# orottier/web-audio-api-rs

Hardware: NVIDIA H100
Metric: offline render-quanta/sec (48kHz stereo, 128-frame) (higher is better)
Workload: dtype f64 filter state / f32 PCM

## Files before the change

web-audio-api-rs_b200/csrc/wae_device.h:

```cpp
#pragma once
#include <cstdint>
#include <vector_types.h>

#include "wae_spatial.h"

namespace wae {

struct BufRef {
    float* p;
    uint32_t stride;
    uint32_t absolute;
    uint8_t* meta;
    uint32_t meta_stride;
    uint32_t meta_pad;
};
constexpr uint8_t WAE_META_SILENT = 0x80;

struct ChunkInfo {
    int64_t f0;
    int32_t nf;
    int32_t sub;
};

struct OscInst {
// ... 330 lines not shown
    float sample_rate;
    int32_t type;
    int32_t ch;
    int32_t pad;
    int32_t* dyn_len;
    BufRef coefs;
};

struct ParamEvDev {
    int32_t type;
    float value;
    double time;
    double aux;
    double cancel_time;
    int32_t has_cancel;
    int32_t values_off, values_len;
    int32_t pad;
};
struct ParamState {
    float intrinsic;
    int32_t head;
    int32_t has_last;
    int32_t override_valid;
    int32_t inited;
    int32_t pad;
    ParamEvDev last;
    ParamEvDev override_ev;
};
struct ParamInst {
    const ParamEvDev* events;
    const float* curves;
    ParamState* state;
    BufRef in;
    BufRef out;
    float def, mn, mx, intrinsic0;
    float sample_rate;
    int32_t n_events;
    int32_t a_rate;
    int32_t has_last0;
    ParamEvDev last0;
};

enum ChainSrc : int32_t { CHAIN_SRC_BUFFER = 0, CHAIN_SRC_ABSN = 1, CHAIN_SRC_OSC = 2, CHAIN_SRC_CONST = 3 };
struct ChainBiquad {
    double b0, b1, b2, a1, a2;
    double* state;
    int32_t coef;
    int32_t pad;
};
constexpr int CHAIN_MAX_BIQUADS = 2;
struct ChainInst {
    int32_t src_kind;
    int32_t ch;
    int32_t n_biquad;
    int32_t has_shaper;
    float g[4];
    int32_t out_dup;
    int32_t shaper_n;
    int32_t shaper_keeps_silence;
    int32_t pad2;
    const float* curve;
    BufRef in;
    AbsnInst absn;
    OscInst osc;
    ConstInst cst;
    BufRef out;
    int64_t limit;
    int64_t end;
    ChainBiquad bq[CHAIN_MAX_BIQUADS];
};

constexpr int CHAIN_MAX_SLABS = 64;
constexpr int CHAIN_MAX_PRE_SLABS = 256;
struct ChainSched {
    int32_t n_slabs;
    int32_t tiles_per_slab;
    int32_t max_ch;
    int32_t slab_stride;
    uint32_t epoch;
    int32_t pre_log2;
    unsigned* ticket;
    double* handoff;
    unsigned* flags;
};
struct ChainAux {
    unsigned* ticket = nullptr;
    double* handoff = nullptr;
    unsigned* flags = nullptr;
    int32_t slab_stride = 0;
    uint32_t epoch = 0;
};

struct VoiceGroup {
    int32_t first;
    int32_t n_voices;
    BufRef out;
    int32_t out_dup;
    int32_t pad;
    int64_t limit;
};

struct ConvInput {
    BufRef in;
    float* prev;
    float2* xring;
    int32_t in_channel;
    int32_t xring_blocks;
    int64_t end;
};
struct ConvPath {
    BufRef out;
    const float2* h;
    float2* y;
    int32_t input;
    int32_t S;
    int32_t out_channel;
    int32_t accumulate;
    int64_t limit;
    int64_t end;
};
struct ConvCmpInst {
    BufRef in;
    ConvInput x;
    ConvPath path;
    int64_t* cursor;
    float* carry;
    float* win;
    int32_t* qmap;
    int64_t* wdesc;
    int32_t in_ch;
    int32_t pad;
};

struct BindItem {
    float* dst;
    const float* src;
    int64_t stride;
    int64_t src_stride;
    int64_t len;
    int32_t channels;
    int32_t pad;
};

struct RespBindItem {
    const float* src;
    float2* h;
    int64_t src_stride;
    int64_t len;
    float sample_rate;
    int32_t channels;
    int32_t S;
    int32_t normalize;
    float scale;
    int32_t m[4];
    int32_t pad;
};

struct CurvePatch {
    int32_t* dst;
    int32_t keeps, other;
};
struct CurveBindItem {
    const float* src;
    float* dst;
    const CurvePatch* patches;
    int32_t n;
    int32_t n_patches;
};

struct WaveBindItem {
    const float* re;
    const float* im;
    float* dst;
// ... 152 lines not shown
```

web-audio-api-rs_b200/csrc/wae_engine.cu:

```cuda
#include "wae_graph.h"
#include "wae_hostmath.h"
#include "wae_hrtf_host.h"
#include "wae_resample_host.h"
#include "wae_kernels.h"
#include "wae_param_core.h"
#include "wae_param_host.h"

#include <cuda.h>
#include <cuda_runtime.h>
#include <emmintrin.h>

#include <algorithm>
#include <array>
#include <atomic>
#include <chrono>
#include <condition_variable>
#include <cstdlib>
#include <deque>
#include <fstream>
#include <mutex>
#include <sched.h>
#include <sstream>
#include <thread>
#include <cmath>
// ... 897 lines not shown
    std::vector<int> out_ch;
    std::vector<BufRef> out_buf;
    std::vector<Lay> out_lay;
    bool wrote_dest = false;
    Lay lay_out(int port) const { return port < (int)out_lay.size() ? out_lay[port] : Lay::fixed(out_ch[port]); }
};

struct NodeTable {
    std::vector<PNode> v;
    std::vector<char> has;
    void reset(uint32_t max_id) {
        if (v.size() < (size_t)max_id + 1) v.resize((size_t)max_id + 1);
        has.assign(v.size(), 0);
    }
    PNode& put(uint32_t id, Node* n) {
        if (id >= v.size()) {
            v.resize((size_t)id + 1);
            has.resize((size_t)id + 1, 0);
        }
        PNode& p = v[id];
        p.n = n;
        p.level = 0;
        p.in_edges.resize((size_t)n->n_inputs);
        for (auto& port : p.in_edges) port.clear();
        p.in_ch.clear();
        p.in_buf.clear();
        p.in_lay.clear();
        p.out_ch.clear();
        p.out_buf.clear();
        p.out_lay.clear();
        p.wrote_dest = false;
        has[id] = 1;
        return p;
    }
    PNode* find(uint32_t id) { return id < v.size() && has[id] ? &v[id] : nullptr; }
    bool count(uint32_t id) const { return id < v.size() && has[id]; }
    PNode& at(uint32_t id) {
        if (!(id < v.size() && has[id])) throw std::out_of_range("planner: unknown node id");
        return v[id];
    }
};

struct Planner {
    wae_batch* b;
    wae_engine* eng;
    Planner(wae_batch* b, const wae_batch::Group& grp, PrepState& ps, std::vector<wae_batch::Group::SrcCopy>* sizing_copies);
    std::map<std::pair<int, int>, StageBuild> builds;
    std::string error;
    int error_code = 0;
    uint64_t algorithmic_bytes = 0;
    struct IrSpectra {
        float2* h;
        int S;
        int channels;
    };
    std::unordered_map<uint64_t, IrSpectra> own_ir_cache;
    std::unordered_map<uint64_t, IrSpectra>* ir_cache = &own_ir_cache;
    std::map<int, std::pair<const float2*, const float2*>> os_filters;

    bool has_feedback = false;
    std::map<std::pair<uint32_t, uint32_t>, int>* delay_ch_hint = nullptr;
    std::map<std::pair<uint32_t, uint32_t>, int> delay_ch_seen;
    struct DelayRing {
        float* ring;
        uint32_t ring_len;
        int ch;
        int64_t* mono_at;
        int32_t mono_len;
    };
    std::map<std::pair<uint32_t, uint32_t>, DelayRing> delay_rings;
    std::map<std::pair<uint32_t, uint32_t>, int> conv_paths_seen;
    bool dry = false;
    int group_graphs = 1;
    int vs_mode = -1;
    int voice_sum_mode() {
        if (eng->voice_sum >= 0) return eng->voice_sum;
        if (vs_mode < 0) {
            const char* e = getenv("WAE_VOICE_SUM");
            vs_mode = e ? std::max(0, std::min(2, atoi(e))) : 0;
        }
        return vs_mode;
    }
    uint64_t arena_floats_per_frame = 0;
    float* d_src = nullptr;
    std::vector<wae_batch::Group::SrcCopy>* src_copies = nullptr;
    size_t src_cursor = 0;
    struct PendingChain {
        ChainInst inst;
        hm::BiquadCoefs coefs[CHAIN_MAX_BIQUADS] = {};
        int ch = 1;
        int phase = 0;
        int cls = 0;
        Lay lay;
        std::vector<Entry> entries;
        Entry gain_fold[4] = {};
        void add_entry(Entry e, size_t off, size_t field) {
            e.refer(0, T_A, -1, off, field);
            entries.push_back(e);
        }
    };

    uint32_t key_graph = 0, key_node = 0, key_seq = 0;
    uint64_t dry_gi = 0, dry_seq = 0;
    uintptr_t dry_addr() { return (uintptr_t)256 + ((dry_gi + 1) << 44) + (dry_seq++ << 24); }
    uint64_t key_salt = 0;
    template <typename T>
    T* alloc(size_t count, bool zero = false, bool rezero_on_run = false) {
        if (dry) return reinterpret_cast<T*>(dry_addr());
        if (seg_start == 0 && seg_end >= lq) return b->dalloc<T>(count, zero, rezero_on_run);
        const wae_batch::StateKey key{key_graph, key_node, key_seq++, key_salt};
        const size_t bytes = count * sizeof(T);
        std::lock_guard<std::recursive_mutex> lk(b->mu);
        auto it = b->state_map.find(key);
        if (it != b->state_map.end() && it->second.second == bytes) return (T*)it->second.first;
        T* p = b->dalloc<T>(count, zero, rezero_on_run);
        if (p) b->state_map[key] = {(void*)p, bytes};
        return p;
    }
    std::map<int, std::vector<float*>> arena_pool;
    std::map<int, size_t> arena_used;
    std::map<std::pair<uint32_t, uint32_t>, size_t> src_offsets;
    std::unordered_map<const PcmBuffer*, size_t> buf_offsets;
    struct ParamRecord {
        size_t n_source_events = 0;
        ParamTimeline tl;
        int64_t init_frame = 0;
    };
    std::unordered_map<uint64_t, ParamRecord> param_records;
    const ParamTimeline* param_timeline(uint32_t gi, uint32_t pid, const Param& prm, float sample_rate) {
        const uint64_t rec_key = (uint64_t)gi << 32 | pid;
        auto it = param_records.find(rec_key);
        if (it == param_records.end()) {
            ParamRecord r;
            r.tl = build_param_timeline(prm);
            r.n_source_events = prm.events.size();
            r.init_frame = seg_start;
            return &param_records.emplace(rec_key, std::move(r)).first->second.tl;
        }
        ParamRecord& r = it->second;
        if (r.n_source_events == prm.events.size() || !r.tl.error.empty()) return &r.tl;
        ParamInst host{};
        host.events = r.tl.events.data();
        host.curves = r.tl.curves.data();
        host.n_events = (int32_t)r.tl.events.size();
        host.a_rate = prm.a_rate ? 1 : 0;
        host.sample_rate = sample_rate;
        ParamState st{};
        st.intrinsic = r.tl.intrinsic;
        st.has_last = r.tl.has_last ? 1 : 0;
        st.last = r.tl.last;
        st.inited = 1;
        float buf[128];
        for (int64_t f = r.init_frame; f < seg_start; f += 128) param_compute_buffer(host, st, (double)f / (double)sample_rate, buf);
        ParamTimeline next;
        next.curves = r.tl.curves;
        for (int i = st.head; i < host.n_events; i++) next.events.push_back(i == st.head && st.override_valid ? st.override_ev : r.tl.events[i]);
        next.intrinsic = st.intrinsic;
        next.has_last = st.has_last != 0;
        next.last = st.last;
        fold_param_events(next, prm.events.data() + r.n_source_events, prm.events.size() - r.n_source_events);
        r.tl = std::move(next);
        r.n_source_events = prm.events.size();
        r.init_frame = seg_start;
        return &r.tl;
    }
    int64_t seg_start = 0, seg_end = 0;
    int64_t lq = 0, glq = 0;
    BufRef dest_ref() const { return BufRef{b->d_out + b->out_off[gi], (uint32_t)g->length, 1}; }
    void add_out(StageBuild& s, size_t off, int t = T_A) const {
        Entry e = entry(E_OUT);
        e.p.out.off = (uint64_t)b->out_off[gi];
        s.add_entry(e, off + offsetof(BufRef, p), offsetof(OutPatch, dst), t);
    }
    int64_t dest_reader = -1;
    void begin_segment(int64_t f0, int64_t f1) {
        seg_start = f0;
        seg_end = f1;
        builds.clear();
        arena_used.clear();
        arena_floats_per_frame = 0;
    }
    template <typename T>
    T* upload(const std::vector<T>& v) {
        if (dry) return reinterpret_cast<T*>(uintptr_t(256));
        return b->dupload(v);
    }

    bool bail(int code, const std::string& msg) {
        if (!error_code) {
            error_code = code;
            error = msg;
        }
        return false;
    }
    bool no_arena() { return bail(WAE_OUT_OF_MEMORY, "out of device memory (arena)"); }

    int cur_cls = 0;
    StageBuild& stage(int level, int kind, int variant = 0) {
        const int cls = cur_cls;
        const int order = kind >= S_READOUT_FFT ? S_ANALYSER * 64 - 3 + (kind - S_READOUT_FFT) : kind * 64 + variant;
        StageBuild& s = builds[{cls * 1000000 + level, order}];
        s.cls = cls;
        s.level = level;
        s.kind = kind;
        s.variant = variant;
        return s;
    }

    BufRef arena_buf(int ch, bool with_meta = false) {
        arena_floats_per_frame += (uint64_t)ch;
        const uint32_t mstride = (uint32_t)((b->chunk / 128 + 16) / 16 * 16);
        BufRef r{dry ? reinterpret_cast<float*>(dry_addr()) : nullptr, (uint32_t)b->chunk, 0, nullptr, 0, 0};
        if (!dry) {
            std::vector<float*>& pool = arena_pool[ch];
            size_t& used = arena_used[ch];
            if (used < pool.size()) {
                r.p = pool[used++];
            } else {
                const size_t floats = (size_t)ch * (size_t)b->chunk;
                float* p = b->dalloc<float>(floats + ((size_t)ch * mstride + 3) / 4);
                b->arena_bytes += floats * 4;
                if (p) {
                    pool.push_back(p);
                    used++;
                }
                r.p = p;
            }
        }
        if (with_meta && r.p) {
            r.meta = reinterpret_cast<uint8_t*>(r.p + (size_t)ch * (size_t)b->chunk);
            r.meta_stride = mstride;
        }
        return r;
    }
    void meta_stage(int L, int mode, const BufRef& in, int in_ch, const BufRef& out, int out_ch, int count = 0, int aux = 0) {
        MetaInst m{};
        m.in = in;
        m.out = out;
        m.mode = mode;
        m.in_ch = in_ch;
        m.out_ch = out_ch;
        m.count = count;
        m.aux = aux;
        stage(L, S_META).meta.push_back(m);
    }

    wae_graph* g = nullptr;
    uint32_t gi = 0;
    Orderer ord{};
    NodeTable node_table;
    SchedClock clock{48000.f};
    bool want_scan_coefs = false;
    std::map<uint32_t, PendingChain> pending;
    struct NodeCtx {
        uint32_t id;
        Node& n;
        PNode& p;
        int level = 0, L = 1;
        Lay in0;
        bool dyn_params = false, fuse_n = false;
        bool extend = false, dest_direct = false;
        uint32_t fuse_src = 0;
    };
// ... 970 lines not shown
        ch = max_in;
    }
    p.in_ch[port] = ch;
    p.in_lay[port] = Lay::fixed(ch);
    bool is_dest = n.kind == K_DEST;
    if (nc.extend || nc.dest_direct) {
        if (nc.extend) p.in_lay[port] = pending.at(nc.fuse_src).lay;
        return true;
    }
    if (vsum_nb >= 0) return sum_voices(nc, port, ch, vsum_nb);
    if (is_dest && edges.size() == 1 && pn.at(edges[0].node).wrote_dest) {
        p.in_buf[port] = pn.at(edges[0].node).out_buf[edges[0].port];
        return true;
    }
    bool any_dyn = false;
    Lay pl = Lay::fixed(ch);
    if (!edges.empty()) {
        int lo = 1, hi = 1, on_nlo = 0, min_nlo = 255;
        bool all_may_silent = true;
        for (auto& r : edges) {
            const Lay el = pn.at(r.node).lay_out(r.port);
            any_dyn = any_dyn || el.dyn();
            lo = std::max<int>(lo, el.lo);
            hi = std::max<int>(hi, el.hi);
            if (!el.may_silent) on_nlo = std::max<int>(on_nlo, el.nlo);
            min_nlo = std::min<int>(min_nlo, el.nlo);
            all_may_silent = all_may_silent && el.may_silent;
        }
        const int nlo = std::max(on_nlo, min_nlo);
        pl.lo = (uint8_t)computed_channels(n.cfg, lo);
        pl.hi = (uint8_t)computed_channels(n.cfg, hi);
        pl.nlo = (uint8_t)computed_channels(n.cfg, nlo);
        pl.nhi = pl.hi;
        pl.may_silent = all_may_silent;
        if (n.kind == K_DELAY_R) pl = pn.at(edges[0].node).lay_out(edges[0].port);
    }
    bool needs_fold = false;
    if (ch > 2 && n.cfg.mode != WAE_COUNT_MODE_EXPLICIT)
        for (auto& r : edges) needs_fold = needs_fold || pn.at(r.node).out_ch[r.port] != ch;
    if (!is_dest && edges.size() == 1 && pn.at(edges[0].node).out_ch[edges[0].port] == ch) {
        const Lay el = pn.at(edges[0].node).lay_out(edges[0].port);
        const bool identity = !el.dyn() || n.kind == K_DELAY_R || n.cfg.mode == WAE_COUNT_MODE_MAX ||
                              (n.cfg.mode == WAE_COUNT_MODE_CLAMPED_MAX && el.hi <= n.cfg.count);
        const bool canonical_needed = el.dyn() && n.kind == K_CONV;
        if (identity && !canonical_needed) {
            p.in_buf[port] = pn.at(edges[0].node).out_buf[edges[0].port];
            p.in_lay[port] = el;
            return true;
        }
    }
    const bool dyn = any_dyn || needs_fold;
    if (!mix(2 * nc.level, edges, ch, n.cfg, is_dest, dyn, dyn && pl.dyn(), p.in_buf[port])) return false;
    if (dyn) p.in_lay[port] = pl;
    return true;
}

bool Planner::sum_voices(NodeCtx& nc, int port, int ch, int nb) {
    auto& edges = nc.p.in_edges[port];
    StageBuild& vs = stage(2 * nc.level, S_VSUM, nb);
    VoiceGroup vg{};
    vg.first = (int32_t)vs.chain.size();
    vg.n_voices = (int32_t)edges.size();
    vg.out_dup = ch;
    vg.limit = -1;
    if (nc.n.kind == K_DEST) {
        vg.out = dest_ref();
        vg.limit = (int64_t)g->length;
    } else {
        vg.out = arena_buf(ch);
        if (!vg.out.p) return no_arena();
    }
    for (auto& r : edges) {
        PendingChain pc = std::move(pending.at(r.node));
        pending.erase(r.node);
        if (pc.inst.n_biquad == 1 && vs.n_scan_coef != vs.chain.size()) return bail(WAE_UNSUPPORTED, "internal: voice-sum coefficient table out of step");
        for (int k = 0; k < pc.inst.n_biquad; k++)
            pc.inst.bq[k].coef = vs.add_scan_coef(want_scan_coefs, [&] { return make_scan_coef(pc.coefs[k]); });
        pc.inst.limit = -1;
        pc.inst.out_dup = 0;
        chain_entries(vs, pc, (int32_t)vs.chain.size());
        vs.chain.push_back(pc.inst);
    }
    vs.vgroups.push_back(vg);
    if (nc.n.kind == K_DEST) add_out(vs, offsetof(VoiceGroup, out), T_C);
    nc.p.in_buf[port] = vg.out;
    return true;
}

bool Planner::lower_dest(NodeCtx& nc) {
    PNode& p = nc.p;
    p.out_ch = {(int)g->channels};
    if (nc.dest_direct) {
        PendingChain pc = std::move(pending.at(nc.fuse_src));
        pending.erase(nc.fuse_src);
        const BufRef fin = dest_ref();
        pc.inst.out = fin;
        pc.inst.limit = (int64_t)g->length;
        pc.inst.out_dup = (pc.ch == 1 && g->channels == 2) ? 2 : 0;
        add_out(emit_chain(pc, nc.L), offsetof(ChainInst, out));
        node_table.at(nc.fuse_src).out_buf = {fin};
        p.in_buf[0] = fin;
    }
    p.out_buf = {p.in_buf[0]};
    if (const std::vector<Edge>* outs = ord.edges.find(nc.id))
        for (auto& e : *outs)
            if (e.other_index >= 0 && dest_reader < 0) dest_reader = gi;
    algorithmic_bytes += (uint64_t)g->channels * g->length * 4;
    return true;
}

bool Planner::lower_osc(NodeCtx& nc) {
    Node& n = nc.n; PNode& p = nc.p;
    const double sr = (double)g->sample_rate;
    PRef pf = param_ref(n.params[0]), pd = param_ref(n.params[1]);
    float freq = pf.v, detune = pd.v;
    if (!nc.fuse_n && !need_out(nc, 1)) return false;
    OscInst o{};
    double start_ratio = 0.;
    if (!nc.fuse_n) o.out = p.out_buf[0];
    o.type = n.type;
    double computed_freq = (double)freq * std::exp2((double)detune / 1200.);
    o.incr = computed_freq / sr;
    o.inv_incr = o.incr != 0. ? 1. / o.incr : 0.;
    o.outside_nyquist = std::fabs(computed_freq) >= sr / 2.;
    o.n_first = std::numeric_limits<int64_t>::max();
    o.n_stop = std::numeric_limits<int64_t>::max();
    o.phase0 = 0.;
    if (n.start_time < 1e300) {
        const OscStart st = osc_start(clock, n.start_time, o.incr, o.outside_nyquist);
        o.n_first = st.n_first;
        o.phase0 = st.phase0;
        start_ratio = st.start_ratio;
        o.n_stop = osc_stop_frame(clock, n.stop_time);
    }
    SchedPatch sched{};
    if (n.device_schedule) sched = sched_entry(n, nc.dyn_params ? SCHED_OSC_AR : SCHED_OSC);
    SchedPatch meta_sched = sched;
    meta_sched.kind = SCHED_META_OSC;
    const SchedPatch* track_sched = n.device_schedule ? &meta_sched : nullptr;
    const bool pitch_bound = pf.bound >= 0 || pd.bound >= 0;
    Entry pitch = patch(PATCH_OSC, 2);
    if (pitch_bound && !nc.dyn_params) {
        const double f_lo = pf.bound >= 0 ? pf.lo : freq, f_hi = pf.bound >= 0 ? pf.hi : freq;
        const double d_lo = pd.bound >= 0 ? pd.lo : detune, d_hi = pd.bound >= 0 ? pd.hi : detune;
        if (!hm::osc_pitch_inside(f_lo, f_hi, d_lo, d_hi, sr)) {
            const uint32_t caller = b->order.empty() ? gi : b->order[gi];
            return bail(WAE_UNSUPPORTED, "graph " + std::to_string(caller) + ", OscillatorNode " + std::to_string(n.id) +
                                             ": the pitch bound from device memory allows computed frequencies outside (0, sampleRate / 2) "
                                             "with frequency [" + std::to_string(f_lo) + ", " + std::to_string(f_hi) + "] Hz and detune [" +
                                             std::to_string(d_lo) + ", " + std::to_string(d_hi) +
                                             "] cents (bind a wider pitch as a value curve: wae_param_set_device_value_curve)");
        }
        operand(pitch, 0, pf, freq);
        operand(pitch, 1, pd, detune);
        pitch.p.param.sample_rate = g->sample_rate;
        double* start = upload(std::vector<double>{n.start_time});
        if (!start) return bail(WAE_OUT_OF_MEMORY, "out of device memory (oscillator start time)");
        pitch.p.param.dst2 = start;
        if (n.device_schedule) sched.start_out = start;
    }
    if (n.type == WAE_OSC_CUSTOM && n.device_wave) {
        o.table = device_wave(n);
        o.table_len = (int)n.device_wave_len;
        if (!o.table) return false;
    } else if (n.type == WAE_OSC_CUSTOM) {
        float* d = upload(n.table);
// ... 1526 lines not shown
    }
    if (uniform) return WAE_OK;
    std::vector<std::vector<int64_t>> cuts(n_graphs);
    for (uint32_t i = 0; i < n_graphs; i++) cuts[i] = graph_cuts(graphs[i]);
    order.resize(n_graphs);
    for (uint32_t i = 0; i < n_graphs; i++) order[i] = i;
    std::stable_sort(order.begin(), order.end(), [&](uint32_t x, uint32_t y) {
        if (graphs[x]->sample_rate != graphs[y]->sample_rate) return graphs[x]->sample_rate < graphs[y]->sample_rate;
        if (cuts[x] != cuts[y]) return cuts[x] < cuts[y];
        return padded_length(graphs[x]) > padded_length(graphs[y]);
    });
    return WAE_OK;
}

static wae_status prep_begin(wae_engine* eng, wae_graph* const* graphs, uint32_t n_graphs, wae_plan_info* plan, wae_batch** out_b, PrepState& ps,
                             bool want_d_out, const std::vector<uint32_t>* order = nullptr) {
    if (!eng || !graphs || n_graphs == 0) return fail(WAE_INVALID_ARGUMENT, "null / empty batch");
    if (!plan) CUDA_TRY(cudaSetDevice(eng->device));
    for (uint32_t i = 0; i < n_graphs; i++) {
        if (!graphs[i]) return fail(WAE_INVALID_ARGUMENT, "null graph in the batch");
        if (!order && (graphs[i]->channels != graphs[0]->channels || graphs[i]->length != graphs[0]->length ||
                       graphs[i]->sample_rate != graphs[0]->sample_rate))
            return fail(WAE_INVALID_ARGUMENT, "all graphs of a batch must share number_of_channels, length and sample_rate");
    }
    ps.t0 = std::chrono::steady_clock::now();
    auto* b = new wae_batch;
    b->engine = eng;
    b->s_h2d = eng->s_h2d;
    b->s_d2h = eng->s_d2h;
    b->n_graphs = n_graphs;
    b->channels = graphs[0]->channels;
    b->out_off.assign(n_graphs + 1, 0);
    for (uint32_t i = 0; i < n_graphs; i++) {
        b->length = std::max(b->length, graphs[i]->length);
        b->out_off[i + 1] = b->out_off[i] + (size_t)graphs[i]->channels * graphs[i]->length;
        b->shape.push_back({graphs[i]->channels, graphs[i]->length});
    }
    b->lq = (int64_t)((b->length + 127) / 128 * 128);
    for (uint32_t i = 0; i < n_graphs; i++) b->needed_quanta += (uint64_t)(padded_length(graphs[i]) / 128);
    if (order) {
        b->mixed = true;
        b->order = *order;
        b->pos.assign(n_graphs, 0);
        for (uint32_t i = 0; i < n_graphs; i++) b->pos[b->order[i]] = i;
    }
    bool has_conv = false, has_hrtf = false;
    std::vector<char> graph_has_conv(n_graphs, 0);
    std::vector<std::vector<int64_t>> cuts(n_graphs);
    for (uint32_t i = 0; i < n_graphs; i++) {
        for (auto& kv : graphs[i]->nodes) {
            if (kv.second.kind == K_CONV && kv.second.buffer) graph_has_conv[i] = 1;
            if (kv.second.kind == K_PANNER && kv.second.panning_model == WAE_PANNING_HRTF) has_hrtf = true;
        }
        cuts[i] = graph_cuts(graphs[i]);
        for (auto& ep : graphs[i]->epochs)
            for (auto& kv : ep.nodes)
                if (kv.second.kind == K_CONV && kv.second.buffer) graph_has_conv[i] = 1;
        has_conv = has_conv || graph_has_conv[i];
    }
    size_t out_floats = b->out_off[n_graphs];
    if (!plan && want_d_out) {
        b->d_out = b->dalloc<float>(out_floats, true);
        if (!b->d_out) {
            wae_batch_destroy(b);
            return fail(WAE_OUT_OF_MEMORY, "out of device memory (output PCM)");
        }
    }
    b->groups = form_groups(eng, graphs, n_graphs, cuts);
    int n_groups = (int)b->groups.size();
    for (auto& grp : b->groups) {
        bool conv = false;
        for (uint32_t i = grp.g0; i < grp.g1; i++) conv = conv || graph_has_conv[i];
        if (!conv) continue;
        for (int64_t f : grp.seg_bounds)
            if (f != grp.lq && f % WAE_CONV_BLOCK != 0) {
                wae_batch_destroy(b);
                return fail(WAE_UNSUPPORTED, "a suspend point that is not a multiple of the convolver partition (8192 frames) in a graph with a ConvolverNode is not lowered to the GPU");
            }
    }
    b->chunk = 2048;
    uint64_t fpf = 0;
    bool has_feedback = false;
    std::vector<std::vector<int>> plan_stage_lists;
    struct SizeOut {
        uint64_t fpf = 0;
        bool has_feedback = false;
        std::map<std::pair<uint32_t, uint32_t>, int> delay_ch_seen;
        std::vector<std::vector<int>> stage_lists;
        uint64_t digest = 1469598103934665603ull, entries_digest = 1469598103934665603ull;
        size_t n_entries = 0;
        int code = WAE_OK;
        std::string error;
    };
    WorkerPool* pool = (!plan && n_groups > 1 && n_graphs >= 64) ? eng->workers() : nullptr;
    bool converged = false;
    for (int iter = 0; iter < 8; iter++) {
        bool hints_changed = false;
        fpf = 0;
        plan_stage_lists.clear();
        std::vector<SizeOut> so(n_groups);
        struct RangeOut {
            uint64_t fpf = 0;
            size_t src_floats = 0;
            bool has_feedback = false;
            std::map<std::pair<uint32_t, uint32_t>, int> delay_ch_seen;
            std::vector<wae_batch::Group::SrcCopy> copies;
            std::vector<size_t> graph_base;
            Builds builds;
            int code = WAE_OK;
            std::string error;
        };
        auto size_range = [&](int k, uint32_t i0, uint32_t i1, RangeOut& ro, size_t cursor0) {
            Planner sizing(b, b->groups[k], ps, &ro.copies);
            sizing.src_cursor = cursor0;
            sizing.begin_segment(0, b->groups[k].lq);
            for (uint32_t i = i0; i < i1; i++) {
                EpochView view(graphs[i], 0);
                ro.graph_base.push_back(sizing.src_cursor);
                if (!sizing.plan_graph(graphs[i], i)) {
                    ro.code = sizing.error_code;
                    ro.error = sizing.error;
                    return;
                }
            }
            if (plan) ro.builds = std::move(sizing.builds);
            ro.fpf = sizing.arena_floats_per_frame;
            ro.src_floats = sizing.src_cursor - cursor0;
            ro.has_feedback = sizing.has_feedback;
            ro.delay_ch_seen = std::move(sizing.delay_ch_seen);
        };
        auto size_group_split = [&](int k, WorkerPool* wp, int parts, RangeOut& out, const std::vector<size_t>* known_base = nullptr) {
            const uint32_t g0 = b->groups[k].g0, n = b->groups[k].g1 - g0;
            std::vector<RangeOut> ro((size_t)parts);
            auto run = [&](int t) {
                const uint32_t i0 = (uint32_t)((uint64_t)n * t / parts), i1 = (uint32_t)((uint64_t)n * (t + 1) / parts);
                size_range(k, g0 + i0, g0 + i1, ro[t], known_base ? (*known_base)[i0] : 0);
            };
            if (wp) wp->parallel_for(parts, run);
            else
                for (int t = 0; t < parts; t++) run(t);
            for (auto& r : ro) {
                if (r.code != WAE_OK) {
                    out.code = r.code;
                    out.error = r.error;
                    return false;
                }
                const size_t rebase = known_base ? 0 : out.src_floats;
                for (auto& c : r.copies) out.copies.push_back(wae_batch::Group::SrcCopy{c.buf, c.offset + rebase, c.floats, c.graph, c.node});
                for (size_t gb : r.graph_base) out.graph_base.push_back(gb + rebase);
                if (plan) merge_builds(out.builds, r.builds);
                out.fpf += r.fpf;
                out.src_floats += r.src_floats;
                out.has_feedback = out.has_feedback || r.has_feedback;
                for (auto& kv : r.delay_ch_seen) out.delay_ch_seen[kv.first] = kv.second;
            }
            return true;
        };
        auto group_nodes = [&](int k) {
            size_t nn = 0;
            for (uint32_t i = b->groups[k].g0; i < b->groups[k].g1; i++) nn += graphs[i]->nodes.size();
            return nn;
        };
        static const bool check_split = [] { const char* e = getenv("WAE_PLAN_PARALLEL"); return e && atoi(e) != 0; }();
        auto size_group = [&](int k) {
            const uint32_t n_in_group = b->groups[k].g1 - b->groups[k].g0;
            const bool one_segment = b->groups[k].seg_bounds.size() == 2;
            if (!plan && !pool && one_segment && n_in_group >= 2 && group_nodes(k) >= 4096) {
                WorkerPool* wp = eng->workers();
                RangeOut out;
                if (!size_group_split(k, wp, (int)std::min<uint32_t>(n_in_group, (uint32_t)wp->size()), out)) {
                    so[k].code = out.code;
                    so[k].error = out.error;
                    return;
                }
                b->groups[k].src_copies = std::move(out.copies);
                b->groups[k].graph_src_base = std::move(out.graph_base);
                b->groups[k].src_floats = out.src_floats;
                so[k].fpf = out.fpf;
                so[k].has_feedback = out.has_feedback;
                so[k].delay_ch_seen = std::move(out.delay_ch_seen);
                return;
            }
            b->groups[k].src_copies.clear();
            b->groups[k].graph_src_base.clear();
            Planner sizing(b, b->groups[k], ps, &b->groups[k].src_copies);
            const std::vector<int64_t>& bounds = b->groups[k].seg_bounds;
            uint64_t serial_digest = 0, serial_entries = 0;
            size_t unused = 0;
            for (size_t sg = 0; sg + 1 < bounds.size(); sg++) {
                sizing.begin_segment(bounds[sg], bounds[sg + 1]);
                for (uint32_t i = b->groups[k].g0; i < b->groups[k].g1; i++) {
                    EpochView view(graphs[i], bounds[sg]);
                    if (one_segment) b->groups[k].graph_src_base.push_back(sizing.src_cursor);
                    if (!sizing.plan_graph(graphs[i], i)) {
                        so[k].code = sizing.error_code;
                        so[k].error = sizing.error;
                        return;
                    }
                }
                so[k].fpf = std::max(so[k].fpf, sizing.arena_floats_per_frame);
                if (plan) {
                    std::vector<int> kinds;
                    for (auto& kv : sizing.builds) kinds.push_back(kv.second.kind);
                    so[k].stage_lists.push_back(std::move(kinds));
                    if (plan_digest_wanted()) {
                        so[k].digest = digest_builds(sizing.builds, so[k].digest);
                        so[k].entries_digest = digest_entries(sizing.builds, so[k].entries_digest, so[k].n_entries);
                    }
                    if (check_split && one_segment) {
                        serial_digest = digest_builds(sizing.builds, 1469598103934665603ull);
                        serial_entries = digest_entries(sizing.builds, 1469598103934665603ull, unused);
                    }
                }
            }
            b->groups[k].src_floats = sizing.src_cursor;
            so[k].has_feedback = sizing.has_feedback;
            so[k].delay_ch_seen = std::move(sizing.delay_ch_seen);
            if (plan && check_split && one_segment && n_in_group >= 2) {
                RangeOut out;
                static const bool threaded = [] { const char* e = getenv("WAE_PLAN_PARALLEL"); return e && atoi(e) >= 2; }();
                std::unique_ptr<WorkerPool> tmp_pool(threaded ? new WorkerPool(3, 0) : nullptr);
                const bool ok = size_group_split(k, tmp_pool.get(), (int)std::min<uint32_t>(n_in_group, 3u), out);
                bool same = ok && out.fpf == so[k].fpf && out.src_floats == b->groups[k].src_floats && out.has_feedback == so[k].has_feedback &&
                            out.delay_ch_seen == so[k].delay_ch_seen && out.copies.size() == b->groups[k].src_copies.size() &&
                            out.graph_base == b->groups[k].graph_src_base;
                if (same) {
                    RangeOut abs_out;
                    same = size_group_split(k, nullptr, (int)std::min<uint32_t>(n_in_group, 3u), abs_out, &b->groups[k].graph_src_base) &&
                           abs_out.graph_base == b->groups[k].graph_src_base && digest_builds(abs_out.builds, 1469598103934665603ull) == serial_digest &&
                           digest_entries(abs_out.builds, 1469598103934665603ull, unused) == serial_entries;
                }
                for (size_t c = 0; same && c < out.copies.size(); c++) {
                    const auto& x = out.copies[c];
                    const auto& y = b->groups[k].src_copies[c];
                    same = x.buf == y.buf && x.offset == y.offset && x.floats == y.floats;
                }
                if (!same) {
                    so[k].code = WAE_INVALID_STATE;
                    so[k].error = "internal: the split sizing pass disagrees with the serial one";
                }
            }
        };
        if (pool) pool->parallel_for(n_groups, size_group);
        else
            for (int k = 0; k < n_groups; k++) size_group(k);
        for (int k = 0; k < n_groups; k++) {
            if (so[k].code != WAE_OK) {
                int code = so[k].code;
                std::string msg = so[k].error;
                wae_batch_destroy(b);
                return fail(code, msg);
            }
            fpf = std::max(fpf, so[k].fpf);
            has_feedback = has_feedback || so[k].has_feedback;
            for (auto& l : so[k].stage_lists) plan_stage_lists.push_back(std::move(l));
            if (plan && plan_digest_wanted()) {
                std::fprintf(stderr, "[wae plan digest] group %d fpf %llu src %zu: %016llx\n", k, (unsigned long long)so[k].fpf, b->groups[k].src_floats, (unsigned long long)so[k].digest);
                std::fprintf(stderr, "[wae plan entries] group %d entries %zu: %016llx\n", k, so[k].n_entries, (unsigned long long)so[k].entries_digest);
            }
            for (auto& kv : so[k].delay_ch_seen) {
                auto it = ps.delay_ch_hint.find(kv.first);
                int cur = it == ps.delay_ch_hint.end() ? 1 : it->second;
                if (cur != kv.second) {
                    ps.delay_ch_hint[kv.first] = kv.second;
                    hints_changed = true;
                }
            }
        }
        if (!hints_changed) {
            converged = true;
            break;
        }
    }
    if (!converged) {
        wae_batch_destroy(b);
        return fail(WAE_UNSUPPORTED, "the channel layout of DelayNodes inside feedback cycles did not settle (graph not lowered to the GPU)");
    }
    ps.t1 = std::chrono::steady_clock::now();
    b->arena_bytes = 0;
    b->asset_bytes = 0;
    int64_t chunk = eng->chunk_frames;
    if (chunk == 0) {
        if (fpf == 0) {
            chunk = b->lq;
        } else {
            chunk = (int64_t)(1024.0 * 1024 * 1024 / (4.0 * (double)fpf));
            chunk = std::max<int64_t>(8192, std::min<int64_t>(chunk, 1 << 20));
            chunk = chunk / 2048 * 2048;
        }
        if (has_conv || has_hrtf) chunk = std::max<int64_t>(chunk, 8 * WAE_CONV_BLOCK);
    }
    (void)has_feedback;
    if (has_conv || has_hrtf) chunk = (chunk + WAE_CONV_BLOCK - 1) / WAE_CONV_BLOCK * WAE_CONV_BLOCK;
    if (chunk > b->lq) chunk = (has_conv || has_hrtf) ? (b->lq + WAE_CONV_BLOCK - 1) / WAE_CONV_BLOCK * WAE_CONV_BLOCK : b->lq;
    b->chunk = chunk;
    if (plan) {
        std::memset(plan, 0, sizeof *plan);
        plan->groups = (uint32_t)n_groups;
        plan->chunk_frames = (uint64_t)chunk;
        plan->chunks = (uint64_t)((b->lq + chunk - 1) / chunk);
        plan->arena_floats_per_frame = fpf;
        plan->has_feedback = has_feedback ? 1u : 0u;
        uint32_t per_kind[S_KINDS] = {0};
        for (auto& grp : b->groups) {
            plan->source_floats += grp.src_floats;
            plan->segments += (uint32_t)grp.seg_bounds.size() - 1;
        }
        for (auto& kinds : plan_stage_lists) {
            plan->stages += (uint32_t)kinds.size();
            for (int k : kinds) per_kind[k]++;
        }
        std::string txt;
        for (int k = 0; k < S_KINDS; k++)
            if (per_kind[k]) txt += (txt.empty() ? "" : ", ") + std::string(kStageNames[k]) + " x " + std::to_string(per_kind[k]);
        std::snprintf(plan->stage_kinds, sizeof plan->stage_kinds, "%s", txt.c_str());
        delete b;
        *out_b = nullptr;
        return WAE_OK;
    }
    for (auto& grp : b->groups) {
        if (cudaEventCreateWithFlags(&grp.ev_h2d, cudaEventDisableTiming) != cudaSuccess ||
            cudaEventCreateWithFlags(&grp.ev_done, cudaEventDisableTiming) != cudaSuccess) {
            const std::string msg = std::string("prepare: cudaEventCreate: ") + cudaGetErrorString(cudaGetLastError());
            wae_batch_destroy(b);
            return fail(WAE_CUDA_ERROR, msg);
        }
        if (grp.src_floats) {
            grp.d_src = b->dalloc<float>(grp.src_floats, false);
            if (!grp.d_src) {
                wae_batch_destroy(b);
                return fail(WAE_OUT_OF_MEMORY, "out of device memory (source PCM slab)");
            }
        }
    }
    *out_b = b;
    return WAE_OK;
}

static void prep_plan_group(wae_batch* b, wae_graph* const* graphs, int k, PrepState& ps, GroupPlan& gp) {
    wae_engine* eng = b->engine;
    wae_batch::Group& grp = b->groups[k];
    Planner pl(b, grp, ps, nullptr);
    auto oom = [&](const char* what) {
        gp.code = WAE_OUT_OF_MEMORY;
        gp.error = std::string("out of device memory (") + what + ")";
    };
    int split_parts = 0;
    {
        static const bool split_on = [] { const char* e = getenv("WAE_PLAN_SPLIT"); return !e || atoi(e) != 0; }();
        const uint32_t n_in_group = grp.g1 - grp.g0;
        size_t nn = 0;
        for (uint32_t i = grp.g0; i < grp.g1; i++) nn += graphs[i]->nodes.size();
        if (split_on && b->groups.size() == 1 && grp.seg_bounds.size() == 2 && n_in_group >= 2 && nn >= 4096 && grp.graph_src_base.size() == n_in_group) {
            const int free_workers = eng->workers()->size() - 1;
            if (free_workers >= 2) split_parts = (int)std::min<uint32_t>(n_in_group, (uint32_t)free_workers);
        }
    }
    for (int sg = 0; sg + 1 < (int)grp.seg_bounds.size(); sg++) {
        pl.begin_segment(grp.seg_bounds[sg], grp.seg_bounds[sg + 1]);
        const uint64_t alg_before = pl.algorithmic_bytes;
        if (split_parts >= 2) {
            struct Run {
                Builds builds;
                uint64_t algorithmic_bytes = 0;
                int64_t dest_reader = -1;
                int code = WAE_OK;
                std::string error;
            };
            std::vector<Run> runs((size_t)split_parts);
// ... 20 lines not shown
                    gp.code = r.code;
                    gp.error = r.error;
                    return;
                }
                merge_builds(pl.builds, r.builds);
                pl.algorithmic_bytes += r.algorithmic_bytes;
                if (pl.dest_reader < 0) pl.dest_reader = r.dest_reader;
            }
        } else
        for (uint32_t i = grp.g0; i < grp.g1; i++) {
            EpochView view(graphs[i], grp.seg_bounds[sg]);
            if (!pl.plan_graph(graphs[i], i)) {
                gp.code = pl.error_code;
                gp.error = pl.error;
                return;
            }
        }
        gp.algorithmic_bytes += (uint64_t)((double)(pl.algorithmic_bytes - alg_before) * (double)(pl.seg_end - pl.seg_start) / (double)grp.lq);
        const size_t seg_stage0 = gp.stages.size();
        void* last_conv_inputs = nullptr;
        for (auto& kv : pl.builds) {
            StageBuild& s = kv.second;
            Stage st;
            st.seg = sg;
            st.cls = s.cls;
            st.kind = s.kind;
            st.variant = s.variant;
            st.group = k;
            st.max_ch = s.max_ch;
            switch (s.kind) {
                case S_MIX: {
                    for (auto& m : s.mix) {
                        bool simple = true, all_mono = m.n_edges > 0;
                        for (int e = 0; e < m.n_edges; e++) {
                            const MixEdge& ed = s.mix_edges[m.edge_offset + e];
                            bool same = ed.src_ch == m.out_ch;
                            bool dup = ed.src_ch == 1 && m.out_ch == 2 && m.interp == WAE_INTERPRETATION_SPEAKERS;
                            if (!(same || dup)) simple = false;
                            if (ed.src_ch != 1) all_mono = false;
                            if (ed.src.absolute || (ed.src.stride & 3) != 0 || (reinterpret_cast<uintptr_t>(ed.src.p) & 15) != 0) simple = false;
                        }
                        m.simple = simple ? 1 : 0;
                        m.all_mono = (simple && all_mono && (m.out_ch == 1 || (m.out_ch == 2 && m.interp == WAE_INTERPRETATION_SPEAKERS))) ? 1 : 0;
                    }
                    st.n = (int)s.mix.size(); st.d_a = up(b, s.mix); st.d_b = up(b, s.mix_edges);
                    for (auto& m : s.mix) st.n_b = std::max(st.n_b, (int)m.n_edges);
                    break;
                }
                case S_MIX_DYN: {
                    for (auto& m : s.mix_dyn) {
                        bool ok = m.out_ch <= 2;
                        for (int e = 0; e < m.n_edges && ok; e++) {
                            const MixEdge& ed = s.mix_edges[m.edge_offset + e];
                            if (ed.src_ch > 2 || ed.src.absolute || (ed.src.stride & 3) != 0 || (reinterpret_cast<uintptr_t>(ed.src.p) & 15) != 0) ok = false;
                        }
                        m.stereo4 = ok ? 1 : 0;
                    }
                    st.n = (int)s.mix_dyn.size(); st.d_a = up(b, s.mix_dyn); st.d_b = up(b, s.mix_edges);
                    break;
                }
                case S_META: st.n = (int)s.meta.size(); st.d_a = up(b, s.meta); break;
                case S_OSC: st.n = (int)s.osc.size(); st.d_a = up(b, s.osc); break;
                case S_CONST: st.n = (int)s.cst.size(); st.d_a = up(b, s.cst); break;
                case S_ABSN: st.n = (int)s.absn.size(); st.d_a = up(b, s.absn); break;
                case S_BIQUAD: st.n = (int)s.biquad.size(); st.d_a = up(b, s.biquad); break;
                case S_CHAIN: {
                    st.n = (int)s.chain.size(); st.d_a = up(b, s.chain); st.d_b = up(b, s.scan_coef);
                    const int nb = (s.variant % 6) / 2;
                    int slabs = 1, tps = 1;
                    int pre_log2 = -1;
                    if (nb > 0) chain_plan_slabs(st.n, st.max_ch, (int)std::min<int64_t>(b->chunk, pl.seg_end - pl.seg_start), nb, &slabs, &tps, &pre_log2);
                    if (slabs > 1) {
                        const size_t slots = (size_t)st.n * st.max_ch * slabs;
                        st.chain.slab_stride = slabs;
                        st.chain.ticket = b->dalloc<unsigned>(1, true);
                        st.chain.flags = b->dalloc<unsigned>(slots, true);
                        st.chain.handoff = b->dalloc<double>(slots * CHAIN_MAX_BIQUADS * 4);
                        if (!st.chain.ticket || !st.chain.flags || !st.chain.handoff) return oom("chain hand-off");
                    }
                    break;
                }
                case S_VSUM: {
                    st.n = (int)s.vgroups.size(); st.d_a = up(b, s.chain); st.d_b = up(b, s.scan_coef); st.d_c = up(b, s.vgroups);
                    const int64_t nf_max = std::min<int64_t>(b->chunk, pl.seg_end - pl.seg_start);
                    const int tiles = (int)((nf_max + 2047) / 2048);
                    st.chain.slab_stride = tiles;
                    st.chain.ticket = b->dalloc<unsigned>(1, true);
                    st.chain.flags = b->dalloc<unsigned>((size_t)st.n * tiles, true);
                    st.chain.handoff = b->dalloc<double>(s.chain.size() * 2 * 4);
                    if (!st.chain.ticket || !st.chain.flags || !st.chain.handoff) return oom("voice-sum hand-off");
                    break;
                }
                case S_PARAM: st.n = (int)s.param.size(); st.d_a = up(b, s.param); break;
                case S_OSC_AR: st.n = (int)s.osc_ar.size(); st.d_a = up(b, s.osc_ar); break;
                case S_BIQUAD_AR: st.n = (int)s.biquad_ar.size(); st.d_a = up(b, s.biquad_ar); break;
                case S_ABSN_SLOW: st.n = (int)s.absn_slow.size(); st.d_a = up(b, s.absn_slow); break;
                case S_IIR: st.n = (int)s.iir.size(); st.d_a = up(b, s.iir); break;
                case S_GAIN: st.n = (int)s.gain.size(); st.d_a = up(b, s.gain); break;
                case S_SHAPER: st.n = (int)s.shaper.size(); st.d_a = up(b, s.shaper); break;
                case S_SPAN: st.n = (int)s.span.size(); st.d_a = up(b, s.span); st.d_b = up(b, s.span_gains); break;
                case S_PAN: st.n = (int)s.pan.size(); st.d_a = up(b, s.pan); break;
                case S_HRTF: st.n = (int)s.hrtf.size(); st.d_a = up(b, s.hrtf); st.max_ch = s.hrtf.empty() ? 0 : s.hrtf[0].L;
                    st.n_b = (int)s.hrtf_sel.size(); st.d_b = up(b, s.hrtf_sel); break;
                case S_PAN_DYN: st.n = (int)s.pan_dyn.size(); st.d_a = up(b, s.pan_dyn); break;
                case S_ABSN_SERIAL: st.n = (int)s.absn_serial.size(); st.d_a = up(b, s.absn_serial); break;
                case S_ABSN_BOUND: st.n = (int)s.absn_bound.size(); st.d_a = up(b, s.absn_bound); break;
                case S_SHAPER_OS: st.n = (int)s.shaper_os.size(); st.d_a = up(b, s.shaper_os); break;
                case S_ROUTE: st.n = (int)s.route.size(); st.d_a = up(b, s.route); break;
                case S_DELAY_MONO:
                case S_DELAY:
                case S_DELAY_WRITE: st.n = (int)s.delay.size(); st.d_a = up(b, s.delay); break;
                case S_COMP:
                    st.n = (int)s.comp.size(); st.d_a = up(b, s.comp);
                    if (!s.comp_ro.empty() && !(st.d_b = up(b, s.comp_ro))) return oom("compressor read-outs");
                    break;
                case S_ANALYSER: st.n = (int)s.analyser.size(); st.d_a = up(b, s.analyser); break;
                case S_READOUT_FFT:
                case S_READOUT_TIME: {
                    std::vector<ReadoutInst> r = s.readout;
                    std::stable_sort(r.begin(), r.end(), [](const ReadoutInst& x, const ReadoutInst& y) { return x.frame < y.frame; });
                    st.n = (int)r.size();
                    st.d_a = up(b, r);
                    for (const ReadoutInst& x : r) {
                        st.frames.push_back(x.frame);
                        st.n_b = std::max(st.n_b, (int)x.fft_size);
                    }
                    break;
                }
                case S_READOUT_SMOOTH:
                    st.n = (int)s.readout_smooth.size();
                    st.d_a = up(b, s.readout_smooth);
                    for (const ReadoutSmoothInst& x : s.readout_smooth) st.n_b = std::max(st.n_b, (int)x.bins);
                    break;
                case S_CONV_FFT: st.n = (int)s.conv_in.size(); st.d_a = up(b, s.conv_in); last_conv_inputs = st.d_a; break;
                case S_CONV_CMP: st.n = (int)s.conv_cmp.size(); st.d_a = up(b, s.conv_cmp); break;
                case S_CONV_MAC:
                case S_CONV_MAC_ACC:
                    st.n = (int)s.conv_path.size();
                    st.d_a = up(b, s.conv_path);
                    st.d_b = last_conv_inputs;
                    break;
            }
            if (st.n > 0) {
                if (!st.d_a) return oom("stage tables");
                gp.stages.push_back(st);
            }
            if (st.n > 0) {
                char* const tables[4] = {nullptr, static_cast<char*>(st.d_a), static_cast<char*>(st.d_b), static_cast<char*>(st.d_c)};
                for (Entry e : s.entries) {
                    for (const FieldRef& r : e.ref)
                        if (r.table != T_NONE) {
                            char* const at = tables[r.table] + (size_t)r.rec * s.record_bytes(r.table) + r.off;
                            std::memcpy(reinterpret_cast<char*>(&e.p) + r.field, &at, sizeof at);
                        }
                    gp.entries.push_back(e);
                }
            }
        }
        std::vector<char> written(grp.g1 - grp.g0, 0);
        for (auto& kv : pl.builds)
            for (const Entry& e : kv.second.entries)
                if (e.kind == E_OUT) written[e.graph - grp.g0] = 1;
        for (uint32_t j = grp.g0; j < grp.g1; j++) {
            const int64_t len = (int64_t)b->shape[j].second, f1 = std::min<int64_t>(pl.seg_end, len);
            if (written[j - grp.g0] || f1 <= pl.seg_start) continue;
            for (uint32_t c = 0; c < b->shape[j].first; c++)
                gp.out_zero.push_back({b->out_off[j] + (size_t)c * (size_t)len + (size_t)pl.seg_start, (size_t)(f1 - pl.seg_start)});
        }
        gp.seg_ranges.push_back({seg_stage0, gp.stages.size()});
    }
    gp.dest_reader = pl.dest_reader;
    b->flush_uploads();
}
// ... 115 lines not shown
                const BindKey& key = t->keys[k];
                const uint32_t caller = b->order.empty() ? key.graph : b->order[key.graph];
                return fail(WAE_INVALID_STATE, std::string(t->kind->noun) + " never bound: graph " + std::to_string(caller) + ", node " +
                                                   std::to_string(key.node) + (key.param == kNodeLevel ? "" : ", param " + std::to_string(key.param)) +
                                                   " (" + t->kind->bind + ")");
            }
    return WAE_OK;
}

static wae_status record_params(wae_batch* b, wae_graph* const* graphs, uint32_t n_graphs, std::vector<GroupPlan>& gps,
                                std::vector<ParamSlotInfo>& info, std::vector<ParamPatch>& patches, std::vector<SpatialPatch>& spatial,
                                std::vector<RespBindItem>& resp) {
    b->params.seal(graphs, n_graphs, [](uint32_t j, const NodeMap& nodes, const Node& nd, auto& declare) {
        if (nd.kind == K_PARAM) return;
        for (uint32_t i = 0; i < nd.params.size(); i++) {
            const Param& prm = nodes.at(nd.params[i]).param;
            if (!prm.device_bound) continue;
            const float def = nd.kind == K_OSC ? std::min(std::max(prm.default_value, prm.device_lo), prm.device_hi) : prm.default_value;
            declare({j, nd.id, i}, DevParam{nd.params[i], ParamSlotInfo{prm.device_lo, prm.device_hi, def, 0}}, false);
        }
    });
    if (b->params.keys.empty()) return WAE_OK;
    std::unordered_map<uint64_t, int32_t> slot_of;
    for (size_t k = 0; k < b->params.keys.size(); k++) {
        slot_of[(uint64_t)b->params.keys[k].graph << 32 | b->params.data[k].pid] = (int32_t)k;
        info.push_back(b->params.data[k].info);
    }
    for (auto& gp : gps)
        for (const Entry& e : gp.entries) {
            if (e.kind != E_PARAM) continue;
            ParamPatch p = e.p.param;
            for (int i = 0; i < PATCH_OPS; i++)
                if (p.slot[i] >= 0) p.slot[i] = slot_of.at((uint64_t)e.graph << 32 | (uint32_t)p.slot[i]);
            patches.push_back(p);
        }
    for (auto& gp : gps)
        for (const Entry& sr : gp.entries) {
            if (sr.kind != E_SPATIAL) continue;
            SpatialPatch p = sr.p.spatial;
            for (int i = 0; i < 15; i++)
                if (p.slot[i] >= 0) p.slot[i] = slot_of.at((uint64_t)sr.graph << 32 | (uint32_t)p.slot[i]);
            spatial.push_back(p);
            b->spatial_sphere = b->spatial_sphere || p.kind != SPATIAL_PAN;
            if (p.kind != SPATIAL_RESP) continue;
            RespBindItem it{};
            it.src = p.resp;
            it.h = sr.spec;
            it.src_stride = it.len = p.taps;
            it.channels = 2;
            it.S = sr.S;
            it.scale = 1.f;
            it.m[0] = it.m[1] = p.taps;
            resp.push_back(it);
            b->spatial_max_taps = std::max(b->spatial_max_taps, p.taps);
            b->spatial_max_S = std::max(b->spatial_max_S, sr.S);
        }
    b->sphere_gen = b->engine->sphere_gen;
    b->n_spatial = (int)spatial.size();
    b->n_spatial_resp = (int)resp.size();
    b->d_spatial = spatial.empty() ? nullptr : b->dupload_now(spatial);
    b->d_spatial_resp = resp.empty() ? nullptr : b->dupload_now(resp);
    if ((!spatial.empty() && !b->d_spatial) || (!resp.empty() && !b->d_spatial_resp))
        return fail(WAE_OUT_OF_MEMORY, "out of device memory (spatial entries)");
    b->d_slot_info = b->dupload_now(info);
    b->d_values = b->dalloc<float>(info.size(), true);
    b->n_patches = (int)patches.size();
    b->d_patches = patches.empty() ? nullptr : b->dupload_now(patches);
    if (!b->d_slot_info || !b->d_values || (!patches.empty() && !b->d_patches)) return fail(WAE_OUT_OF_MEMORY, "out of device memory (bound params)");
    return WAE_OK;
}

static wae_status prep_finish(wae_batch* b, PrepState& ps) {
    CUDA_TRY(cudaEventCreate(&b->ev0));
    CUDA_TRY(cudaEventCreate(&b->ev1));
    int64_t n_chunks = 0;
    for (auto& grp : b->groups)
    {
        int64_t c = 0;
        for (size_t sg = 0; sg + 1 < grp.seg_bounds.size(); sg++) c += (grp.seg_bounds[sg + 1] - grp.seg_bounds[sg] + b->chunk - 1) / b->chunk;
        n_chunks = std::max(n_chunks, c);
    }
    uint64_t launches = 0;
    for (auto& st : b->stages) {
        const uint64_t k = (st.kind == S_CONV_FFT || st.kind == S_CONV_MAC || st.kind == S_CONV_MAC_ACC || st.kind == S_SHAPER_OS) ? 2
                           : st.kind == S_HRTF ? (st.n_b > 0 ? 3 : 2) : st.kind == S_CONV_CMP ? 6 : 1;
        const std::vector<int64_t>& sb = b->groups[st.group].seg_bounds;
        const int64_t seg_len = sb[st.seg + 1] - sb[st.seg];
        launches += st.cls == 1 ? k * (uint64_t)(seg_len / 128) : k * (uint64_t)((seg_len + b->chunk - 1) / b->chunk);
    }
    std::memset(&b->stats, 0, sizeof(b->stats));
    b->stats.kernel_launches_per_run = launches;
    b->stats.stages = b->stages.size();
    b->stats.chunks = (uint64_t)n_chunks;
    b->stats.arena_bytes = b->arena_bytes;
    b->stats.asset_bytes = b->asset_bytes;
    b->stats.algorithmic_bytes = ps.algorithmic_bytes;
    b->stats.graph_quanta = b->needed_quanta;
    return WAE_OK;
}

static wae_status alloc_readout_rows(wae_batch* b, wae_graph* const* graphs, uint32_t n_graphs) {
    for (uint32_t c = 0; c < n_graphs; c++) {
        const uint32_t j = b->batch_pos(c);
        if (!graphs[j]->analyser_readouts && !graphs[j]->compressor_readouts) continue;
        for (const auto& kv : graphs[j]->nodes) {
            const Node& n = kv.second;
            if (n.kind == K_COMP && !n.readout_q.empty()) b->comp_readout_outs[kv.first].add(n_graphs, j, n.readout_q.size());
            if (n.kind != K_ANALYSER || !n.readout_kinds) continue;
            for (uint32_t kind : {(uint32_t)WAE_READOUT_FREQUENCY, (uint32_t)WAE_READOUT_TIME_DOMAIN}) {
                if (!(n.readout_kinds & kind)) continue;
                const uint64_t elems = (uint64_t)n.readout_q.size() * (kind == WAE_READOUT_FREQUENCY ? n.fft_size / 2 : n.fft_size);
                b->readout_outs[{kv.first, kind}].add(n_graphs, j, elems);
                if (n.byte_readout_kinds & kind) b->byte_readout_outs[{kv.first, kind}].add(n_graphs, j, elems);
            }
        }
    }
    for (auto& kv : b->readout_outs)
        if (!(kv.second.d = b->dalloc<float>(kv.second.count))) return fail(WAE_OUT_OF_MEMORY, "out of device memory (analyser read-outs)");
    for (auto& kv : b->byte_readout_outs)
        if (!(kv.second.d = b->dalloc<uint8_t>(kv.second.count))) return fail(WAE_OUT_OF_MEMORY, "out of device memory (analyser read-outs)");
    for (auto& kv : b->comp_readout_outs)
        if (!(kv.second.d = b->dalloc<float>(kv.second.count, true))) return fail(WAE_OUT_OF_MEMORY, "out of device memory (compressor read-outs)");
    return WAE_OK;
}

static wae_status prepare_impl(wae_engine* eng, wae_graph* const* graphs, uint32_t n_graphs, wae_batch** out, wae_plan_info* plan,
                               const std::vector<uint32_t>* order = nullptr) {
    if (!out && !plan) return fail(WAE_INVALID_ARGUMENT, "null out pointer");
    PrepState ps;
    wae_batch* b = nullptr;
    wae_status st = prep_begin(eng, graphs, n_graphs, plan, &b, ps, true, order);
    if (st != WAE_OK || plan) return st;
    record_device_inputs(b, graphs, n_graphs);
    st = alloc_readout_rows(b, graphs, n_graphs);
    if (st != WAE_OK) {
        wae_batch_destroy(b);
        return st;
    }
    const int n_groups = (int)b->groups.size();
    std::vector<GroupPlan> gps(n_groups);
    WorkerPool* pool = (n_groups > 1 && n_graphs >= 64) ? eng->workers() : nullptr;
    if (pool) pool->parallel_for(n_groups, [&](int k) { prep_plan_group(b, graphs, k, ps, gps[k]); });
    else
        for (int k = 0; k < n_groups; k++) prep_plan_group(b, graphs, k, ps, gps[k]);
    for (int k = 0; k < n_groups; k++) {
        if (gps[k].code != WAE_OK) {
            int code = gps[k].code;
            std::string msg = gps[k].error;
            wae_batch_destroy(b);
            return fail(code, msg);
        }
        prep_append_group(b, k, ps, gps[k]);
        wae_status cs = enqueue_source_copies(b, b->groups[k], eng->stream);
        if (cs != WAE_OK) {
            wae_batch_destroy(b);
            return cs;
        }
    }
    std::vector<CurvePatch> curve_patches;
    std::vector<IirPatch> iir_patches;
    std::vector<SchedPatch> sched_patches;
    std::vector<LoopPatch> loop_patches;
    std::vector<LoopWalk> loop_walks;
    std::vector<SrcRefPatch> src_refs;
    std::vector<ParamSlotInfo> slot_info;
    std::vector<ParamPatch> patches;
    std::vector<SpatialPatch> spatial;
// ... 39 lines not shown

WAE_API wae_status wae_batch_plan(wae_graph* const* graphs, uint32_t n_graphs, wae_plan_info* info) {
    if (!info) return fail(WAE_INVALID_ARGUMENT, "null info pointer");
    wae_engine host_only;
    return prepare_impl(&host_only, graphs, n_graphs, nullptr, info);
}

struct ManyOrder {
    std::vector<uint32_t> order;
    std::vector<wae_graph*> sorted;
    wae_graph* const* graphs = nullptr;
    const std::vector<uint32_t>* order_ptr() const { return order.empty() ? nullptr : &order; }
};
static wae_status many_batch(wae_graph* const* graphs, uint32_t n_graphs, ManyOrder& mo) {
    wae_status st = many_order(graphs, n_graphs, mo.order);
    if (st != WAE_OK) return st;
    mo.graphs = graphs;
    if (!mo.order.empty()) {
        for (uint32_t i : mo.order) mo.sorted.push_back(graphs[i]);
        mo.graphs = mo.sorted.data();
    }
    return WAE_OK;
}

WAE_API wae_status wae_batch_prepare_many(wae_engine* eng, wae_graph* const* graphs, uint32_t n_graphs, wae_batch** out) {
    if (!out) return fail(WAE_INVALID_ARGUMENT, "null out pointer");
    ManyOrder mo;
    wae_status st = many_batch(graphs, n_graphs, mo);
    if (st != WAE_OK) return st;
    return prepare_impl(eng, mo.graphs, n_graphs, out, nullptr, mo.order_ptr());
}

WAE_API wae_status wae_batch_plan_many(wae_graph* const* graphs, uint32_t n_graphs, wae_plan_info* info) {
    if (!info) return fail(WAE_INVALID_ARGUMENT, "null info pointer");
    ManyOrder mo;
    wae_status st = many_batch(graphs, n_graphs, mo);
    if (st != WAE_OK) return st;
    wae_engine host_only;
    return prepare_impl(&host_only, mo.graphs, n_graphs, nullptr, info, mo.order_ptr());
}

WAE_API wae_status wae_batch_plan_quanta(wae_graph* const* graphs, uint32_t n_graphs, uint32_t* group_of, uint64_t* rendered, uint64_t* needed) {
    if (!rendered || !needed) return fail(WAE_INVALID_ARGUMENT, "null argument");
    ManyOrder mo;
    wae_status st = many_batch(graphs, n_graphs, mo);
    if (st != WAE_OK) return st;
    wae_engine host_only;
    std::vector<std::vector<int64_t>> cuts(n_graphs);
    for (uint32_t i = 0; i < n_graphs; i++) cuts[i] = graph_cuts(mo.graphs[i]);
    const std::vector<wae_batch::Group> groups = form_groups(&host_only, mo.graphs, n_graphs, cuts);
    *rendered = *needed = 0;
    for (size_t k = 0; k < groups.size(); k++)
        for (uint32_t j = groups[k].g0; j < groups[k].g1; j++) {
            *rendered += (uint64_t)(groups[k].lq / 128);
            *needed += (uint64_t)(padded_length(mo.graphs[j]) / 128);
            if (group_of) group_of[mo.order.empty() ? j : mo.order[j]] = (uint32_t)k;
        }
    return WAE_OK;
}

static void launch_stage(wae_batch* b, Stage& st, ChunkInfo ci) {
    cudaStream_t s = b->engine->stream;
    switch (st.kind) {
        case S_MIX: launch_mix((MixInst*)st.d_a, (MixEdge*)st.d_b, st.n, ci, s, st.n_b); break;
        case S_MIX_DYN: launch_mix_dyn((MixDynInst*)st.d_a, (MixEdge*)st.d_b, st.n, ci, s); break;
        case S_META: launch_meta((MetaInst*)st.d_a, st.n, ci, s); break;
        case S_DELAY_MONO: launch_delay_mono((DelayInst*)st.d_a, st.n, ci, s); break;
        case S_OSC: launch_oscillator((OscInst*)st.d_a, st.n, ci, s); break;
        case S_CONST: launch_constant((ConstInst*)st.d_a, st.n, ci, s); break;
        case S_ABSN: launch_buffer_source((AbsnInst*)st.d_a, st.n, ci, s); break;
        case S_BIQUAD:
            launch_biquad_serial((BiquadInst*)st.d_a, st.n, st.max_ch, ci, s);
            break;
        case S_PARAM: launch_param((ParamInst*)st.d_a, st.n, ci, s, b->engine->param_parallel); break;
        case S_OSC_AR: launch_osc_arate((OscArInst*)st.d_a, st.n, ci, s); break;
        case S_ABSN_SLOW: launch_buffer_source_slow((AbsnSlowInst*)st.d_a, st.n, ci, s); break;
        case S_BIQUAD_AR: launch_biquad_arate((BiquadArInst*)st.d_a, st.n, st.max_ch, ci, s); break;
        case S_CHAIN:
            st.chain.epoch++;
            launch_chain(st.variant, (ChainInst*)st.d_a, (ScanCoef*)st.d_b, st.n, st.max_ch, ci, s, st.chain);
            break;
        case S_VSUM:
            st.chain.epoch++;
            launch_voice_sum(st.variant, (ChainInst*)st.d_a, (ScanCoef*)st.d_b, (VoiceGroup*)st.d_c, st.n, ci, s, st.chain);
            break;
        case S_IIR: launch_iir((IirInst*)st.d_a, st.n, st.max_ch, ci, s); break;
        case S_GAIN: launch_gain((GainInst*)st.d_a, st.n, ci, s); break;
        case S_SHAPER: launch_shaper((ShaperInst*)st.d_a, st.n, ci, s); break;
        case S_SPAN: launch_stereo_panner((SPanInst*)st.d_a, (float2*)st.d_b, st.n, ci, s); break;
        case S_PAN: launch_panner_eq((PanInst*)st.d_a, st.n, ci, s); break;
        case S_HRTF: launch_hrtf((HrtfInst*)st.d_a, st.n, (HrtfSelInst*)st.d_b, st.n_b, st.max_ch, ci, s); break;
        case S_PAN_DYN: launch_panner_dyn((PanDynInst*)st.d_a, st.n, ci, s); break;
        case S_ABSN_SERIAL: launch_buffer_source_serial((AbsnSerialInst*)st.d_a, st.n, ci, s); break;
        case S_ABSN_BOUND: launch_buffer_source_bound((AbsnBoundInst*)st.d_a, st.n, ci, s); break;
        case S_SHAPER_OS: launch_shaper_os((ShaperOsInst*)st.d_a, st.n, st.max_ch, ci, s); break;
        case S_ROUTE: launch_route((RouteInst*)st.d_a, st.n, ci, s); break;
        case S_DELAY: launch_delay_read((DelayInst*)st.d_a, st.n, ci, s); break;
        case S_DELAY_WRITE: launch_ring_write((DelayInst*)st.d_a, st.n, ci, s); break;
        case S_COMP: launch_compressor((CompInst*)st.d_a, (const CompReadoutInst*)st.d_b, st.n, ci, s); break;
        case S_ANALYSER: launch_analyser((AnalyserInst*)st.d_a, st.n, ci, s); break;
        case S_READOUT_FFT:
        case S_READOUT_TIME: {
            const int64_t lo = ci.f0 == 0 ? -1 : ci.f0;
            const size_t r0 = std::upper_bound(st.frames.begin(), st.frames.end(), lo) - st.frames.begin();
            const size_t r1 = std::upper_bound(st.frames.begin(), st.frames.end(), ci.f0 + ci.nf) - st.frames.begin();
            if (r1 <= r0) break;
            const ReadoutInst* d = (const ReadoutInst*)st.d_a + r0;
            if (st.kind == S_READOUT_FFT) launch_readout_fft(d, (int)(r1 - r0), st.n_b, ci, s);
            else launch_readout_time(d, (int)(r1 - r0), st.n_b, ci, s);
            break;
        }
        case S_READOUT_SMOOTH: launch_readout_smooth((ReadoutSmoothInst*)st.d_a, st.n, st.n_b, ci, s); break;
        case S_CONV_FFT: launch_conv_fft_in((ConvInput*)st.d_a, st.n, ci, s); break;
        case S_CONV_MAC:
        case S_CONV_MAC_ACC: launch_conv_mac_ifft((ConvPath*)st.d_a, (ConvInput*)st.d_b, st.n, ci, s); break;
        case S_CONV_CMP: launch_conv_compact((ConvCmpInst*)st.d_a, st.n, ci, s); break;
    }
}

static bool group_sources_pinned(const wae_batch::Group& g) {
    for (auto& sc : g.src_copies)
        if (!sc.buf->device_input && !sc.buf->pinned) return false;
    return true;
}
static wae_status ensure_host_mirror(wae_batch* b) {
    for (auto& g : b->groups) {
        if (!g.src_floats || g.h_src || group_sources_pinned(g)) continue;
        void* hp = nullptr;
        if (cudaHostAlloc(&hp, g.src_floats * sizeof(float), cudaHostAllocDefault) != cudaSuccess) {
            cudaGetLastError();
            return fail(WAE_OUT_OF_MEMORY, "out of memory (pinned mirror of the source PCM)");
        }
        b->pinned.push_back(hp);
        g.h_src = (float*)hp;
        for (auto& sc : g.src_copies)
            if (!sc.buf->device_input) std::memcpy(g.h_src + sc.offset, sc.buf->base, sc.floats * sizeof(float));
    }
    return WAE_OK;
}
static wae_status resend_group_sources(wae_batch* b, wae_batch::Group& g, cudaStream_t s) {
    if (!g.src_floats) return WAE_OK;
    if (g.h_src && !g.has_device_inputs) {
        CUDA_TRY(cudaMemcpyAsync(g.d_src, g.h_src, g.src_floats * sizeof(float), cudaMemcpyHostToDevice, s));
        return WAE_OK;
    }
    if (g.h_src) {
        size_t i = 0;
        const auto& cs = g.src_copies;
        while (i < cs.size()) {
            if (cs[i].buf->device_input) {
                i++;
                continue;
            }
            size_t j = i + 1, end = cs[i].offset + cs[i].floats;
            while (j < cs.size() && !cs[j].buf->device_input && cs[j].offset == end) end += cs[j++].floats;
            CUDA_TRY(cudaMemcpyAsync(g.d_src + cs[i].offset, g.h_src + cs[i].offset, (end - cs[i].offset) * sizeof(float), cudaMemcpyHostToDevice, s));
            i = j;
        }
        return WAE_OK;
    }
    return enqueue_source_copies(b, g, s);
}

WAE_API wae_status wae_batch_upload(wae_batch* b) {
    CUDA_TRY(cudaSetDevice(b->engine->device));
    wae_status ms = ensure_host_mirror(b);
    if (ms != WAE_OK) return ms;
// ... 1218 lines not shown
```

web-audio-api-rs_b200/csrc/wae_kernels.cu:

```cuda
#include "wae_kernels.h"
#include "wae_param_core.h"
#include "wae_param_walk.h"
#include "../../include/wae.h"

#include <algorithm>
#include <cmath>
#include <cstdlib>
#include <vector>
#include <type_traits>
#include <cuda_runtime.h>
#include <math_constants.h>

namespace wae {

#define DEVI __device__ __forceinline__

DEVI float* chan(const BufRef& b, int c, const ChunkInfo& ci) { return b.p + (size_t)c * b.stride + (b.absolute ? ci.f0 : ci.sub); }

DEVI int meta_qi(const ChunkInfo& ci, int n) { return (ci.sub + n) >> 7; }
DEVI bool buf_silent(const BufRef& b, int rows, int qi) {
    if (!b.meta) return false;
    for (int r = 0; r < rows; r++)
        if (!(b.meta[(size_t)r * b.meta_stride + qi] & WAE_META_SILENT)) return false;
    return true;
// ... 999 lines not shown
#pragma unroll
                    for (int j = 0; j < CH_K; j++) {
                        v[j] = __ll2float_rn((long long)ph) * 1.08420217248550443e-19f;
                        if ((unsigned)((ph + cw) >> 32) <= thr) mask |= 1u << j;
                        asm("add.u64 %0, %0, %1;" : "+l"(ph) : "l"(dph));
                    }
                    while (mask) {
                        const int jw = __ffs((int)mask) - 1;
                        mask &= mask - 1;
                        const unsigned long long pj = ph0 + (unsigned long long)jw * dph;
                        const float sw = osc_saw_blep(pj + HALF, inc, inv);
#pragma unroll
                        for (int j = 0; j < CH_K; j++) v[j] = j == jw ? sw : v[j];
                    }
                } else {
                    const bool wide = dph >= 0x4000000000000000ull;
#pragma unroll
                    for (int j = 0; j < CH_K; j++) {
                        v[j] = (long long)ph >= 0 ? 1.0f : -1.0f;
                        if (((unsigned)((ph + dph) >> 32) & 0x7fffffffu) <= thr) mask |= 1u << j;
                        asm("add.u64 %0, %0, %1;" : "+l"(ph) : "l"(dph));
                    }
                    if (wide) mask = (1u << CH_K) - 1u;
                    while (mask) {
                        const int jw = __ffs((int)mask) - 1;
                        mask &= mask - 1;
                        const unsigned long long pj = ph0 + (unsigned long long)jw * dph;
                        const float sw = osc_square_blep(pj, pj + HALF, inc, inv);
#pragma unroll
                        for (int j = 0; j < CH_K; j++) v[j] = j == jw ? sw : v[j];
                    }
                }
            } else {
#pragma unroll
                for (int j = 0; j < CH_K; j++) {
                    long long q = (long long)(ph - 0x4000000000000000ull);
                    q = q < 0 ? -q : q;
                    v[j] = __ll2float_rn((long long)(0x4000000000000000ull - (unsigned long long)q)) * 2.16840434497100887e-19f;
                    asm("add.u64 %0, %0, %1;" : "+l"(ph) : "l"(dph));
                }
            }
        } else {
#pragma unroll
            for (int j = 0; j < CH_K; j++) {
                int64_t n = na + j;
                float s = 0.f;
                if (n >= o.n_first && n < o.n_stop && !o.outside_nyquist) s = osc_sample(o, osc_phase_at(o, n), o.incr);
                v[j] = s;
            }
        }
    } else {
        const ConstInst& o = q.cst;
#pragma unroll
        for (int j = 0; j < CH_K; j++) {
            int64_t n = ci.f0 + n0 + j;
            v[j] = (n >= o.n_first && n < o.n_stop) ? o.value : 0.f;
        }
    }
}

template <int SRC>
__device__ __noinline__ void chain_stage_gather(const ChainInst* q, int c, ChunkInfo ci, int n0, float4* region, int lane, int xq) {
    float tmp[CH_K];
    chain_load_source<SRC>(*q, c, ci, n0, tmp);
#pragma unroll
    for (int u = 0; u < CH_K / 4; u++) region[4 * lane + (u ^ xq)] = make_float4(tmp[4 * u], tmp[4 * u + 1], tmp[4 * u + 2], tmp[4 * u + 3]);
}

struct ChainSmem {
    ChainInst q;
    double state[CHAIN_MAX_BIQUADS][4];
    double P[CHAIN_MAX_BIQUADS][24];
    double plane[CHAIN_MAX_BIQUADS][32][4];
    double wtot[CH_WARPS][2];
    double replay[4];
    float edge[CH_WARPS][2];
    int flushed;
};

struct NoReload {};
template <typename RL>
DEVI void chain_biquad(ChainSmem& sm, int bq, const double b0, const double b1, const double b2, const double a1, const double a2,
                       const double* Plane, float v[CH_K], bool active, int n_active, int t, int lane, int warp, bool want_clean, bool& clean,
                       RL reload) {
    const double* Psh = sm.P[bq];
    const double* Pw = sm.P[bq] + 20;
    const float xl1 = active ? v[CH_K - 1] : 0.f, xl2 = active ? v[CH_K - 2] : 0.f;
    if (lane == 31) {
        sm.edge[warp][0] = xl1;
        sm.edge[warp][1] = xl2;
    }
    const float p1 = __shfl_up_sync(0xffffffffu, xl1, 1);
    const float p2 = __shfl_up_sync(0xffffffffu, xl2, 1);
    __syncthreads();
    double x1, x2;
    if (lane == 0) {
        if (warp == 0) {
            x1 = sm.state[bq][0];
            x2 = sm.state[bq][1];
        } else {
            x1 = (double)sm.edge[warp - 1][0];
            x2 = (double)sm.edge[warp - 1][1];
        }
    } else {
        x1 = (double)p1;
        x2 = (double)p2;
    }
    const bool x_normal = want_clean && (isnormal_d(x1) || isnormal_d(x2));
    double w[CH_K];
    double r1 = 0., r2 = 0.;
    const double na1 = -a1, na2 = -a2;
#pragma unroll
    for (int j = 0; j < CH_K; j++) {
        const double x = (double)v[j];
        w[j] = fma(b2, x2, fma(b1, x1, b0 * x));
        const double y = fma(na1, r1, fma(na2, r2, w[j]));
        x2 = x1;
        x1 = x;
        r2 = r1;
        r1 = y;
    }
    double va = active ? r1 : 0., vb = active ? r2 : 0.;
#pragma unroll
    for (int d = 0; d < 5; d++) {
        const double oa = __shfl_up_sync(0xffffffffu, va, 1 << d);
        const double ob = __shfl_up_sync(0xffffffffu, vb, 1 << d);
        if (lane >= (1 << d)) mat2_fma(Psh + 4 * d, oa, ob, va, vb);
    }
    if (lane == 31) {
        sm.wtot[warp][0] = va;
        sm.wtot[warp][1] = vb;
    }
    const double ea = __shfl_up_sync(0xffffffffu, va, 1);
    const double eb = __shfl_up_sync(0xffffffffu, vb, 1);
    __syncthreads();
    double wa = sm.state[bq][2], wb = sm.state[bq][3];
#pragma unroll
    for (int k = 0; k < CH_WARPS - 1; k++) {
        if (k < warp) {
            double ta = sm.wtot[k][0], tb = sm.wtot[k][1];
            mat2_fma(Pw, wa, wb, ta, tb);
            wa = ta;
            wb = tb;
        }
    }
    double e1 = wa, e2 = wb;
    if (lane != 0) {
        e1 = ea;
        e2 = eb;
        mat2_fma(Plane, wa, wb, e1, e2);
    }
    if (want_clean) clean = !(x_normal || isnormal_d(e1) || isnormal_d(e2));
    r1 = e1;
    r2 = e2;
#pragma unroll
    for (int j = 0; j < CH_K; j++) {
        const double y = fma(na1, r1, fma(na2, r2, w[j]));
        r2 = r1;
        r1 = y;
        v[j] = (float)y;
    }
    const bool last = active && t == n_active - 1;
    const bool poisoned = last && (!(fabs(r1) <= 1.7976931348623157e308) || !(fabs(r2) <= 1.7976931348623157e308));
#ifdef WAE_CHAIN_NOCHECK
    __syncthreads();
    if (false) {
#else
    if (__syncthreads_or(poisoned)) {
#endif
        if (t == 0) sm.flushed = 1;
        if constexpr (!std::is_same<RL, NoReload>::value) {
            float x[CH_K];
            reload(x);
            double sx1 = sm.state[bq][0], sx2 = sm.state[bq][1], sy1 = sm.state[bq][2], sy2 = sm.state[bq][3];
            __syncthreads();
#pragma unroll 1
            for (int wv = 0; wv < CH_WARPS; wv++) {
                if (warp == wv) {
#pragma unroll 1
                    for (int l = 0; l < 32; l++) {
                        double qx1 = sx1, qx2 = sx2, qy1 = sy1, qy2 = sy2;
                        if (lane == l && active) {
#pragma unroll
                            for (int j = 0; j < CH_K; j++) {
                                const double xi = (double)x[j];
                                double y = __dsub_rn(__dsub_rn(__dadd_rn(__dadd_rn(__dmul_rn(b0, xi), __dmul_rn(b1, qx1)), __dmul_rn(b2, qx2)), __dmul_rn(a1, qy1)),
                                                     __dmul_rn(a2, qy2));
                                if (!isnormal_d(y)) y = 0.;
                                qx2 = qx1;
                                qx1 = xi;
                                qy2 = qy1;
                                qy1 = y;
                                v[j] = (float)y;
                            }
                        }
                        sx1 = __shfl_sync(0xffffffffu, qx1, l);
                        sx2 = __shfl_sync(0xffffffffu, qx2, l);
                        sy1 = __shfl_sync(0xffffffffu, qy1, l);
                        sy2 = __shfl_sync(0xffffffffu, qy2, l);
                    }
                    if (lane == 0) {
                        sm.replay[0] = sx1;
                        sm.replay[1] = sx2;
                        sm.replay[2] = sy1;
                        sm.replay[3] = sy2;
                    }
                }
                __syncthreads();
                sx1 = sm.replay[0];
                sx2 = sm.replay[1];
                sy1 = sm.replay[2];
                sy2 = sm.replay[3];
                __syncthreads();
            }
            if (t == 0) {
                sm.state[bq][0] = sx1;
                sm.state[bq][1] = sx2;
                sm.state[bq][2] = sy1;
                sm.state[bq][3] = sy2;
            }
            return;
        } else {
            if (last) r1 = r2 = 0.;
        }
    }
    if (last) {
        sm.state[bq][0] = (double)xl1;
        sm.state[bq][1] = (double)xl2;
        sm.state[bq][2] = r1;
        sm.state[bq][3] = r2;
    }
}

DEVI unsigned smem_u32(const void* p) { return (unsigned)__cvta_generic_to_shared(p); }
DEVI void mbar_init(uint64_t* bar, unsigned count) { asm volatile("mbarrier.init.shared::cta.b64 [%0], %1;" ::"r"(smem_u32(bar)), "r"(count) : "memory"); }
DEVI void mbar_expect_tx(uint64_t* bar, unsigned bytes) {
    asm volatile("mbarrier.arrive.expect_tx.shared::cta.b64 _, [%0], %1;" ::"r"(smem_u32(bar)), "r"(bytes) : "memory");
}
DEVI void mbar_wait(uint64_t* bar, unsigned parity) {
    unsigned ok;
    do {
        asm volatile(
            "{\n"
            ".reg .pred p;\n"
            "mbarrier.try_wait.parity.shared::cta.b64 p, [%1], %2;\n"
            "selp.u32 %0, 1, 0, p;\n"
            "}\n"
            : "=r"(ok)
            : "r"(smem_u32(bar)), "r"(parity)
            : "memory");
    } while (!ok);
}
DEVI void bulk_load(void* smem_dst, const void* gsrc, unsigned bytes, uint64_t* bar) {
    asm volatile("cp.async.bulk.shared::cluster.global.mbarrier::complete_tx::bytes [%0], [%1], %2, [%3];" ::"r"(smem_u32(smem_dst)), "l"(gsrc),
                 "r"(bytes), "r"(smem_u32(bar))
                 : "memory");
}
DEVI void bulk_store(void* gdst, const void* smem_src, unsigned bytes) {
    asm volatile("cp.async.bulk.global.shared::cta.bulk_group [%0], [%1], %2;" ::"l"(gdst), "r"(smem_u32(smem_src)), "r"(bytes) : "memory");
}
DEVI void bulk_commit() { asm volatile("cp.async.bulk.commit_group;" ::: "memory"); }
template <int N>
DEVI void bulk_wait_read() { asm volatile("cp.async.bulk.wait_group.read %0;" ::"n"(N) : "memory"); }
DEVI void fence_proxy_async_smem() { asm volatile("fence.proxy.async.shared::cta;" ::: "memory"); }

#ifndef WAE_CH_STAGES
#define WAE_CH_STAGES 4
#endif
constexpr int CH_STAGES = WAE_CH_STAGES;

DEVI void cswap4(bool p, float4& a, float4& b) {
    const float4 ta = a, tb = b;
    a.x = p ? tb.x : ta.x; a.y = p ? tb.y : ta.y; a.z = p ? tb.z : ta.z; a.w = p ? tb.w : ta.w;
    b.x = p ? ta.x : tb.x; b.y = p ? ta.y : tb.y; b.z = p ? ta.z : tb.z; b.w = p ? ta.w : tb.w;
}

#ifndef WAE_CH_MINB
#define WAE_CH_MINB 6
#endif
#ifndef WAE_CH_MINB_OSC
#define WAE_CH_MINB_OSC 5
#endif
constexpr int chain_min_blocks(int src, int nb) {
    const int base = src == CHAIN_SRC_OSC ? WAE_CH_MINB_OSC : WAE_CH_MINB;
    return ((nb == 2 ? base - 1 : base) * 128) / CH_THREADS;
}
template <int SRC, int NB, bool SHAPER, bool TMA, bool PRE = false>
__global__ void __launch_bounds__(CH_THREADS, chain_min_blocks(SRC, NB)) k_chain(const ChainInst* __restrict__ insts, const ScanCoef* __restrict__ coefs,
                                                                        int n_inst, ChunkInfo ci, ChainSched sc) {
    __shared__ ChainSmem sm;
    __shared__ int s_item;
    const int t = threadIdx.x, lane = t & 31, warp = t >> 5;
    int item = (int)blockIdx.x;
    if (NB > 0 && sc.ticket != nullptr) {
        if (t == 0) {
            const unsigned tk = atomicAdd(sc.ticket, 1u);
            if (tk == gridDim.x - 1) atomicExch(sc.ticket, 0u);
            s_item = (int)tk;
        }
        __syncthreads();
        item = s_item;
    }
    const int per_slab = n_inst * sc.max_ch;
    const int slab = item / per_slab;
    const int rem = item - slab * per_slab;
    const int c = rem / n_inst;
    const int inst = rem - c * n_inst;
    {
        const int* src = reinterpret_cast<const int*>(insts + inst);
        int* dst = reinterpret_cast<int*>(&sm.q);
        for (int i = t; i < (int)(sizeof(ChainInst) / 4); i += CH_THREADS) dst[i] = src[i];
    }
    __syncthreads();
    if (ci.f0 + (int64_t)slab * sc.tiles_per_slab * (CH_THREADS * CH_K) >= sm.q.end && sm.q.out.meta == nullptr) return;
    __shared__ float2 s_table2[SRC == CHAIN_SRC_OSC ? 2048 : 1];
    const float2* tab2 = nullptr;
    if (SRC == CHAIN_SRC_OSC && sm.q.osc.table_len == 2048 && (sm.q.osc.type == 0 || sm.q.osc.type == 4)) {
        const float* gt = sm.q.osc.table;
        for (int i = t; i < 2048; i += CH_THREADS) s_table2[i] = make_float2(__ldg(gt + i), __ldg(gt + ((i + 1) & 2047)));
        tab2 = s_table2;
        __syncthreads();
    }
    const ChainInst& q = sm.q;
    if (c >= q.ch) return;
    constexpr int tile = CH_THREADS * CH_K;
    const int n_tiles = (ci.nf + tile - 1) / tile;
    const int tile0 = slab * sc.tiles_per_slab;
    if (tile0 >= n_tiles) return;
    const int slab_begin = tile0 * tile;
    const int slab_end = min(ci.nf, (tile0 + sc.tiles_per_slab) * tile);
    const bool first_slab = slab == 0, last_slab = slab_end >= ci.nf;
    const size_t ho = ((size_t)inst * sc.max_ch + c) * sc.slab_stride + slab;
    double cb[NB > 0 ? NB : 1][5];
    const bool pre = PRE && NB == 1 && sc.pre_log2 >= 0 && !last_slab;
    auto wait_handoff = [&]() {
        if (t == 0) {
            const unsigned* f = sc.flags + ho;
            unsigned seen;
            for (;;) {
                asm volatile("ld.acquire.gpu.global.u32 %0, [%1];" : "=r"(seen) : "l"(f) : "memory");
                if (seen == sc.epoch) break;
                __nanosleep(256);
            }
        }
        __syncthreads();
    };
    if (NB > 0 && !first_slab && !pre) wait_handoff();
#pragma unroll
    for (int k = 0; k < NB; k++) {
        const ChainBiquad& bq = q.bq[k];
        cb[k][0] = bq.b0; cb[k][1] = bq.b1; cb[k][2] = bq.b2; cb[k][3] = bq.a1; cb[k][4] = bq.a2;
        const ScanCoef& scf = coefs[bq.coef];
        if (t < 20) sm.P[k][t] = (&scf.Pshfl[0][0])[t];
        if (t < 4) {
            sm.P[k][20 + t] = scf.Pwarp[t];
            sm.state[k][t] = pre ? 0. : (first_slab ? bq.state[4 * c + t] : __ldcg(sc.handoff + ho * (CHAIN_MAX_BIQUADS * 4) + 4 * k + t));
        }
        for (int i = t; i < 128; i += CH_THREADS) (&sm.plane[k][0][0])[i] = (&scf.Plane[0][0])[i];
    }
    const float g0 = q.g[0], g1 = q.g[1], g2 = q.g[2], g3 = q.g[3];

    constexpr bool STREAMED = SRC == CHAIN_SRC_BUFFER || SRC == CHAIN_SRC_ABSN;
    constexpr bool USE_TMA = TMA && STREAMED;
    constexpr int NST = STREAMED ? CH_STAGES : 1;
    constexpr int WF = 32 * CH_K / 4;
    __shared__ __align__(128) float4 s_io[NST][CH_WARPS][WF];
    __shared__ __align__(8) uint64_t s_bar[USE_TMA ? NST : 1];
    const int lane_sw = lane ^ ((lane >> 3) & 3);
    const int xq = (lane >> 1) & 3;
    const int wbase = warp * 32 * CH_K;
// ... 12 lines not shown
    if (STREAMED) {
        if (SRC == CHAIN_SRC_BUFFER) {
            const float* p0 = chan(q.in, c, ci) + wbase;
            if ((reinterpret_cast<uintptr_t>(p0) & 15) == 0) {
                s_ptr0 = p0;
                s_lo = 0;
                s_hi = ci.nf - wbase - 32 * CH_K;
            }
        } else {
            const AbsnInst& o = q.absn;
            const long long off = (long long)ci.f0 + wbase - o.n_start + o.buf_offset;
            const float* p0 = o.buf + (size_t)c * o.buf_stride + off;
            if (!o.loop && (reinterpret_cast<uintptr_t>(p0) & 15) == 0) {
                s_ptr0 = p0;
                s_lo = clamp_i(max(0ll, (long long)o.n_start - ci.f0 - wbase));
                s_hi = clamp_i(min((long long)ci.nf - wbase - 32 * CH_K, (long long)o.buf_len - 32 * CH_K - off));
            }
        }
    }
    auto region_src = [&](int tile_base) -> const float* {
        return (tile_base >= s_lo && tile_base <= s_hi) ? s_ptr0 + tile_base : nullptr;
    };
    const int n_out = q.out_dup > 1 ? q.out_dup : 1;
    float* const o_ptr0 = chan(q.out, q.out_dup > 1 ? 0 : c, ci) + wbase;
    int o_hi = ci.nf - wbase - 32 * CH_K;
    if (q.limit >= 0) o_hi = clamp_i(min((long long)o_hi, (long long)q.limit - ci.f0 - wbase - 32 * CH_K));
    if ((reinterpret_cast<uintptr_t>(o_ptr0) & 15) != 0 || (q.out_dup > 1 && (q.out.stride & 3) != 0)) o_hi = -1;
    auto stage_source = [&](int buf, int tile_base) {
        if (!STREAMED || tile_base >= slab_end) return;
        const int nw = tile_base + wbase;
        if (nw >= ci.nf) return;
        const float* gp = region_src(tile_base);
        if (gp) {
#pragma unroll
            for (int u = 0; u < CH_K / 4; u++) {
                const int f = 32 * u + lane;
                const unsigned dst = smem_u32(&s_io[buf][warp][32 * u + lane_sw]);
                asm volatile("cp.async.cg.shared.global [%0], [%1], 16;" ::"r"(dst), "l"(gp + 4 * f) : "memory");
            }
        } else if (nw + lane * CH_K < ci.nf) {
            chain_stage_gather<SRC>(&sm.q, c, ci, nw + lane * CH_K, &s_io[buf][warp][0], lane, xq);
        }
    };
    auto tile_src = [&](int tile_base) -> const float* {
        if (!STREAMED || tile_base + tile > ci.nf) return nullptr;
        if (SRC == CHAIN_SRC_BUFFER) {
            const float* gp = chan(q.in, c, ci) + tile_base;
            return (reinterpret_cast<uintptr_t>(gp) & 15) == 0 ? gp : nullptr;
        } else {
            const AbsnInst& o = q.absn;
            const float* src = o.buf + (size_t)c * o.buf_stride;
            const int64_t n = ci.f0 + tile_base;
            const int64_t idx = n - o.n_start + o.buf_offset;
            if (!o.loop && n >= o.n_start && idx + tile <= o.buf_len && ((reinterpret_cast<uintptr_t>(src + idx) & 15) == 0)) return src + idx;
            return nullptr;
        }
    };
    auto issue_bulk = [&](int buf, int tile_base) {
        if (tile_base >= slab_end) return;
        const float* gp = tile_src(tile_base);
        if (gp) {
            mbar_expect_tx(&s_bar[buf], tile * 4);
            bulk_load(&s_io[buf][0][0], gp, tile * 4, &s_bar[buf]);
        }
    };
    unsigned par = 0;
    auto run_slab = [&](const bool emit) {
    float v[CH_K];
    if (STREAMED) {
        if (USE_TMA) {
            if (t == 0)
#pragma unroll
                for (int s = 0; s < NST - 1; s++) issue_bulk(s, slab_begin + s * tile);
        } else {
#pragma unroll
            for (int s = 0; s < NST - 1; s++) {
                stage_source(s, slab_begin + s * tile);
                asm volatile("cp.async.commit_group;" ::: "memory");
            }
        }
    }
    int buf = 0;
    for (int base = slab_begin; base < slab_end; base += tile) {
        const int n0 = base + t * CH_K;
        const bool active = n0 < ci.nf;
        const int n_active = min(CH_THREADS, (ci.nf - base) / CH_K);
        const int pbuf = buf == 0 ? NST - 1 : buf - 1;
        if (STREAMED && !USE_TMA) {
            stage_source(pbuf, base + (NST - 1) * tile);
            asm volatile("cp.async.commit_group;" ::: "memory");
            asm volatile("cp.async.wait_group %0;" ::"n"(NST - 1) : "memory");
            __syncwarp();
            if (active) {
#pragma unroll
                for (int u = 0; u < CH_K / 4; u++) {
                    const float4 a = s_io[buf][warp][4 * lane + (u ^ xq)];
                    v[4 * u] = a.x; v[4 * u + 1] = a.y; v[4 * u + 2] = a.z; v[4 * u + 3] = a.w;
                }
            }
        } else if (USE_TMA) {
            if (tile_src(base) != nullptr) {
                mbar_wait(&s_bar[buf], (par >> buf) & 1u);
                par ^= 1u << buf;
                float4 a[CH_K / 4];
#pragma unroll
                for (int u = 0; u < CH_K / 4; u++) a[u] = s_io[buf][warp][4 * lane + (u ^ xq)];
                cswap4((xq & 1) != 0, a[0], a[1]);
                cswap4((xq & 1) != 0, a[2], a[3]);
                cswap4((xq & 2) != 0, a[0], a[2]);
                cswap4((xq & 2) != 0, a[1], a[3]);
#pragma unroll
                for (int u = 0; u < CH_K / 4; u++) {
                    v[4 * u] = a[u].x; v[4 * u + 1] = a[u].y; v[4 * u + 2] = a[u].z; v[4 * u + 3] = a[u].w;
                }
            } else if (active) {
                chain_load_source<SRC>(q, c, ci, n0, v, tab2);
            }
        } else if (active) {
            chain_load_source<SRC>(q, c, ci, n0, v, tab2);
        }
        bool clean0 = true, clean1 = true;
        const bool want_clean = q.out.meta != nullptr;
        if (g0 != 1.f) {
#pragma unroll
            for (int j = 0; j < CH_K; j++) v[j] *= g0;
        }
        if (NB >= 1) {
            if constexpr (STREAMED) {
                auto reload = [&](float x[CH_K]) {
                    float4 a[CH_K / 4];
#pragma unroll
                    for (int u = 0; u < CH_K / 4; u++) a[u] = s_io[buf][warp][4 * lane + (u ^ xq)];
                    if (USE_TMA) {
                        cswap4((xq & 1) != 0, a[0], a[1]);
                        cswap4((xq & 1) != 0, a[2], a[3]);
                        cswap4((xq & 2) != 0, a[0], a[2]);
                        cswap4((xq & 2) != 0, a[1], a[3]);
                    }
#pragma unroll
                    for (int u = 0; u < CH_K / 4; u++) {
                        x[4 * u] = a[u].x * g0; x[4 * u + 1] = a[u].y * g0; x[4 * u + 2] = a[u].z * g0; x[4 * u + 3] = a[u].w * g0;
                    }
                };
                chain_biquad(sm, 0, cb[0][0], cb[0][1], cb[0][2], cb[0][3], cb[0][4], sm.plane[0][lane > 0 ? lane - 1 : 0], v, active, n_active, t, lane, warp, want_clean, clean0, reload);
            } else {
                chain_biquad(sm, 0, cb[0][0], cb[0][1], cb[0][2], cb[0][3], cb[0][4], sm.plane[0][lane > 0 ? lane - 1 : 0], v, active, n_active, t, lane, warp, want_clean, clean0, NoReload{});
            }
            if (g1 != 1.f) {
#pragma unroll
                for (int j = 0; j < CH_K; j++) v[j] *= g1;
            }
        }
        if (NB >= 2) {
            chain_biquad(sm, 1, cb[NB - 1][0], cb[NB - 1][1], cb[NB - 1][2], cb[NB - 1][3], cb[NB - 1][4], sm.plane[1][lane > 0 ? lane - 1 : 0], v, active,
                         n_active, t, lane, warp, want_clean, clean1, NoReload{});
            if (g2 != 1.f) {
#pragma unroll
                for (int j = 0; j < CH_K; j++) v[j] *= g2;
            }
        }
        if (SHAPER) {
            const float* curve = q.curve;
            const int cn = q.shaper_n;
            if (curve) {
#pragma unroll
                for (int j = 0; j < CH_K; j++) v[j] = cn == 0 ? 0.f : shaper_apply(curve, cn, v[j]);
            }
#pragma unroll
            for (int j = 0; j < CH_K; j++) v[j] *= g3;
        }
        if (emit && q.out.meta && active && (n0 & 127) == 0) {
            const int qi = meta_qi(ci, n0);
            const int64_t f = ci.f0 + n0;
            bool sl;
            int cnt = q.ch;
            if (SRC == CHAIN_SRC_BUFFER) {
                sl = buf_silent(q.in, q.ch, qi);
                cnt = buf_count(q.in, q.ch, qi);
            } else if (SRC == CHAIN_SRC_OSC) {
                sl = q.osc.n_stop <= f || q.osc.n_first >= f + 128;
            } else if (SRC == CHAIN_SRC_CONST) {
                sl = q.cst.n_stop <= f || q.cst.n_first >= f + 128;
            } else {
                sl = q.absn.n_stop <= f || q.absn.n_start >= f + 128;
            }
            if (g0 == 0.f) sl = true;
            if (sl) cnt = 1;
            if (NB >= 1) {
                if (sl && !clean0) {
                    sl = false;
                    cnt = q.ch;
                }
                if (g1 == 0.f) sl = true;
                if (sl) cnt = 1;
            }
            if (NB >= 2) {
                if (sl && !clean1) {
                    sl = false;
                    cnt = q.ch;
                }
                if (g2 == 0.f) sl = true;
                if (sl) cnt = 1;
            }
            if (SHAPER) {
                if (sl && q.curve && !q.shaper_keeps_silence) sl = false;
                if (g3 == 0.f) sl = true;
            }
            meta_put(q.out, c, qi, cnt, sl || c >= cnt);
        }
        if (emit) {
            const int nw = base + wbase;
            const bool tile_out = USE_TMA && base + tile <= ci.nf && (q.limit < 0 || ci.f0 + base + tile <= q.limit) &&
                                  (reinterpret_cast<uintptr_t>(chan(q.out, q.out_dup > 1 ? 0 : c, ci) + base) & 15) == 0 &&
                                  (q.out_dup <= 1 || (q.out.stride & 3) == 0);
            if (USE_TMA) {
                if (tile_out) {
                    float4 a[CH_K / 4];
#pragma unroll
                    for (int u = 0; u < CH_K / 4; u++) a[u] = make_float4(v[4 * u], v[4 * u + 1], v[4 * u + 2], v[4 * u + 3]);
                    cswap4((xq & 2) != 0, a[0], a[2]);
                    cswap4((xq & 2) != 0, a[1], a[3]);
                    cswap4((xq & 1) != 0, a[0], a[1]);
                    cswap4((xq & 1) != 0, a[2], a[3]);
#pragma unroll
                    for (int u = 0; u < CH_K / 4; u++) s_io[buf][warp][4 * lane + (u ^ xq)] = a[u];
                    fence_proxy_async_smem();
                } else if (active) {
                    const int64_t nabs = ci.f0 + n0;
                    for (int oc = 0; oc < n_out; oc++) {
                        float* out = chan(q.out, q.out_dup > 1 ? oc : c, ci) + n0;
#pragma unroll
                        for (int j = 0; j < CH_K; j++)
                            if (q.limit < 0 || nabs + j < q.limit) out[j] = v[j];
                    }
                }
                __syncthreads();
                if (t == 0) {
                    if (tile_out)
                        for (int oc = 0; oc < n_out; oc++) bulk_store(chan(q.out, q.out_dup > 1 ? oc : c, ci) + base, &s_io[buf][0][0], tile * 4);
                    bulk_commit();
                    bulk_wait_read<1>();
                    issue_bulk(pbuf, base + (NST - 1) * tile);
                }
            } else if (base <= o_hi) {
                __syncwarp();
#pragma unroll
                for (int u = 0; u < CH_K / 4; u++)
                    s_io[buf][warp][4 * lane + (u ^ xq)] = make_float4(v[4 * u], v[4 * u + 1], v[4 * u + 2], v[4 * u + 3]);
                __syncwarp();
                for (int oc = 0; oc < n_out; oc++) {
                    float4* out = reinterpret_cast<float4*>(o_ptr0 + (size_t)oc * q.out.stride + base);
#pragma unroll
                    for (int u = 0; u < CH_K / 4; u++) {
                        out[32 * u + lane] = s_io[buf][warp][32 * u + lane_sw];
                    }
                }
                __syncwarp();
            } else if (active) {
                const int64_t nabs = ci.f0 + n0;
                for (int oc = 0; oc < n_out; oc++) {
                    float* out = chan(q.out, q.out_dup > 1 ? oc : c, ci) + n0;
#pragma unroll
                    for (int j = 0; j < CH_K; j++)
                        if (q.limit < 0 || nabs + j < q.limit) out[j] = v[j];
                }
            }
        }
        if (NB > 0 && !USE_TMA) __syncthreads();
        buf = buf + 1 == NST ? 0 : buf + 1;
    }
    if (STREAMED && !USE_TMA) asm volatile("cp.async.wait_group 0;" ::: "memory");
    };
    if constexpr (PRE && NB == 1 && !TMA) {
        if (pre) {
            if (t == 0) sm.flushed = 0;
            __syncthreads();
            run_slab(false);
            __syncthreads();
            if (!first_slab) wait_handoff();
            if (t == 0) {
                double sin_[4], g[16], h[16];
                const ScanCoef& scf = coefs[q.bq[0].coef];
                for (int i = 0; i < 4; i++) sin_[i] = first_slab ? q.bq[0].state[4 * c + i] : __ldcg(sc.handoff + ho * (CHAIN_MAX_BIQUADS * 4) + i);
                for (int i = 0; i < 16; i++) g[i] = scf.GL[i];
                for (int sq = 0; sq < sc.pre_log2; sq++) {
                    for (int r = 0; r < 4; r++)
                        for (int cc = 0; cc < 4; cc++) {
                            double a = 0.;
                            for (int k = 0; k < 4; k++) a = fma(g[4 * r + k], g[4 * k + cc], a);
                            h[4 * r + cc] = a;
                        }
                    for (int i = 0; i < 16; i++) g[i] = h[i];
                }
                for (int r = 0; r < 4; r++) {
                    double o = sm.state[0][r];
                    if (!sm.flushed)
                        for (int k = 0; k < 4; k++) o = fma(g[4 * r + k], sin_[k], o);
                    __stcg(sc.handoff + (ho + 1) * (CHAIN_MAX_BIQUADS * 4) + r, o);
                }
                __threadfence();
                asm volatile("st.release.gpu.global.u32 [%0], %1;" ::"l"(sc.flags + ho + 1), "r"(sc.epoch) : "memory");
                for (int i = 0; i < 4; i++) sm.state[0][i] = sin_[i];
            }
            __syncthreads();
        }
    }
    run_slab(true);
    if (USE_TMA && t == 0) bulk_wait_read<0>();
    if (NB > 0) {
        if (last_slab) {
#pragma unroll
            for (int k = 0; k < NB; k++)
                if (t < 4) q.bq[k].state[4 * c + t] = sm.state[k][t];
        } else if (!pre) {
            if (t < 4 * NB) __stcg(sc.handoff + (ho + 1) * (CHAIN_MAX_BIQUADS * 4) + t, sm.state[t >> 2][t & 3]);
            __threadfence();
            __syncthreads();
            if (t == 0) asm volatile("st.release.gpu.global.u32 [%0], %1;" ::"l"(sc.flags + ho + 1), "r"(sc.epoch) : "memory");
        }
    }
}

#ifndef WAE_VS_MINB
#define WAE_VS_MINB 5
#endif
template <int NB>
__global__ void __launch_bounds__(CH_THREADS, WAE_VS_MINB * 128 / CH_THREADS) k_voice_sum(const ChainInst* __restrict__ insts, const ScanCoef* __restrict__ coefs,
                                                                                          const VoiceGroup* __restrict__ groups, int n_groups, ChunkInfo ci,
                                                                                          ChainSched sc) {
    __shared__ ChainSmem sm;
    __shared__ int s_item;
    __shared__ float2 s_table2[2048];
    const int t = threadIdx.x, lane = t & 31, warp = t >> 5;
    if (t == 0) {
        const unsigned tk = atomicAdd(sc.ticket, 1u);
        if (tk == gridDim.x - 1) atomicExch(sc.ticket, 0u);
        s_item = (int)tk;
    }
    __syncthreads();
    const int item = s_item;
    const int slab = item / n_groups, gi = item - slab * n_groups;
    const VoiceGroup grp = groups[gi];
    constexpr int tile = CH_THREADS * CH_K;
    const int base = slab * tile;
    if (base >= ci.nf) return;
    const int n0 = base + t * CH_K;
    const bool active = n0 < ci.nf;
    const int n_active = min(CH_THREADS, (ci.nf - base) / CH_K);
    const bool first_slab = slab == 0, last_slab = base + tile >= ci.nf;
    const unsigned tag = (sc.epoch & 0xfffu) << 20;
    const unsigned* prog_prev = sc.flags + (size_t)gi * sc.slab_stride + (slab > 0 ? slab - 1 : 0);
    unsigned* prog_mine = sc.flags + (size_t)gi * sc.slab_stride + slab;
    unsigned seen = 0;
    const float* cur_table = nullptr;
    float acc[CH_K];
#pragma unroll
    for (int j = 0; j < CH_K; j++) acc[j] = 0.f;
    constexpr int REC_W = (int)(sizeof(ChainInst) / 4 + CH_THREADS - 1) / CH_THREADS;
    constexpr int PL_W = (128 + CH_THREADS - 1) / CH_THREADS;
    static_assert(CH_THREADS >= 24, "scan constants: one of Pshfl / Pwarp per thread");
    int rec_n[REC_W];
    double pl_n[PL_W], pw_n = 0.;
    auto prefetch = [&](int vi) {
        const int inst = grp.first + vi;
        const int* src = reinterpret_cast<const int*>(insts + inst);
#pragma unroll
        for (int i = 0; i < REC_W; i++) rec_n[i] = (t + i * CH_THREADS) < (int)(sizeof(ChainInst) / 4) ? __ldg(src + t + i * CH_THREADS) : 0;
        if (NB > 0) {
            const ScanCoef& scf = coefs[inst];
#pragma unroll
            for (int i = 0; i < PL_W; i++) pl_n[i] = (t + i * CH_THREADS) < 128 ? (&scf.Plane[0][0])[t + i * CH_THREADS] : 0.;
            if (t < 20) pw_n = (&scf.Pshfl[0][0])[t];
            else if (t < 24) pw_n = scf.Pwarp[t - 20];
        }
    };
    prefetch(0);
    const bool handoff_in = NB > 0 && !first_slab, handoff_out = NB > 0 && !last_slab;
    auto poll_ok = [&](unsigned x, int v) { return (x & 0xfff00000u) == tag && (x & 0xfffffu) > (unsigned)v; };
    double st_next = 0.;
    bool st_next_valid = false;
    constexpr int PUB_T = CH_WARPS > 1 ? 32 : 0;
    double pe0 = 0., pe1 = 0., pe2 = 0., pe3 = 0.;
    double* pub_ptr = nullptr;
    int pub_vi = -1;
    auto publish = [&]() {
        if (pub_vi < 0) return;
        if (last_slab) {
            pub_ptr[0] = pe0; pub_ptr[1] = pe1; pub_ptr[2] = pe2; pub_ptr[3] = pe3;
        } else {
            double* dst = sc.handoff + ((size_t)(grp.first + pub_vi) * 2 + ((slab + 1) & 1)) * 4;
            asm volatile("st.global.cg.v2.f64 [%0], {%1, %2};" ::"l"(dst), "d"(pe0), "d"(pe1) : "memory");
            asm volatile("st.global.cg.v2.f64 [%0], {%1, %2};" ::"l"(dst + 2), "d"(pe2), "d"(pe3) : "memory");
            asm volatile("st.release.gpu.global.u32 [%0], %1;" ::"l"(prog_mine), "r"(tag | (unsigned)(pub_vi + 1)) : "memory");
        }
        pub_vi = -1;
    };
    for (int vi = 0; vi < grp.n_voices; vi++) {
        const int inst = grp.first + vi;
#pragma unroll
        for (int i = 0; i < REC_W; i++)
            if ((t + i * CH_THREADS) < (int)(sizeof(ChainInst) / 4)) reinterpret_cast<int*>(&sm.q)[t + i * CH_THREADS] = rec_n[i];
        if (NB > 0) {
#pragma unroll
            for (int i = 0; i < PL_W; i++)
                if ((t + i * CH_THREADS) < 128) (&sm.plane[0][0][0])[t + i * CH_THREADS] = pl_n[i];
            if (t < 24) sm.P[0][t] = pw_n;
        }
        __syncthreads();
        if (vi + 1 < grp.n_voices) prefetch(vi + 1);
        const ChainInst& q = sm.q;
        double st_cur = 0.;
        unsigned xa = 0;
        if (NB > 0 && t == PUB_T) publish();
        if (NB > 0 && warp == 0) {
            if (st_next_valid) {
                st_cur = st_next;
            } else if (first_slab) {
                if (lane < 4) st_cur = q.bq[0].state[lane];
            } else {
                if (lane == 0 && seen <= (unsigned)vi) {
                    for (;;) {
                        unsigned x;
                        asm volatile("ld.relaxed.gpu.global.u32 %0, [%1];" : "=r"(x) : "l"(prog_prev) : "memory");
                        if (poll_ok(x, vi)) {
                            seen = x & 0xfffffu;
                            break;
                        }
                        __nanosleep(20);
                    }
                }
                __syncwarp();
                if (lane < 4) st_cur = __ldcg(sc.handoff + ((size_t)inst * 2 + (slab & 1)) * 4 + lane);
            }
            if (handoff_in && lane == 0 && vi + 1 < grp.n_voices && seen <= (unsigned)(vi + 1))
                asm volatile("ld.relaxed.gpu.global.u32 %0, [%1];" : "=r"(xa) : "l"(prog_prev));
        }
        const float2* tab2 = nullptr;
        if ((q.osc.type == 0 || q.osc.type == 4) && q.osc.table_len == 2048) {
            if (q.osc.table != cur_table) {
                const float* gt = q.osc.table;
                for (int i = t; i < 2048; i += CH_THREADS) s_table2[i] = make_float2(__ldg(gt + i), __ldg(gt + ((i + 1) & 2047)));
                cur_table = gt;
                __syncthreads();
            }
            tab2 = s_table2;
        }
        double cb[5] = {0., 0., 0., 0., 0.};
        double* st_ptr = nullptr;
        if (NB > 0) {
            const ChainBiquad& bq = q.bq[0];
            cb[0] = bq.b0; cb[1] = bq.b1; cb[2] = bq.b2; cb[3] = bq.a1; cb[4] = bq.a2;
            st_ptr = bq.state;
        }
        const float g0 = q.g[0], g1 = q.g[1];
        float v[CH_K];
        if (active) chain_load_source<CHAIN_SRC_OSC>(q, 0, ci, n0, v, tab2);
        if (g0 != 1.f) {
#pragma unroll
            for (int j = 0; j < CH_K; j++) v[j] *= g0;
        }
        if (NB > 0) {
            if (warp == 0 && lane < 4) sm.state[0][lane] = st_cur;
            bool clean = true;
            chain_biquad(sm, 0, cb[0], cb[1], cb[2], cb[3], cb[4], sm.plane[0][lane > 0 ? lane - 1 : 0], v, active, n_active, t, lane, warp, false, clean, NoReload{});
            if (g1 != 1.f) {
#pragma unroll
                for (int j = 0; j < CH_K; j++) v[j] *= g1;
            }
        }
        if (active) {
            if (vi == 0) {
#pragma unroll
                for (int j = 0; j < CH_K; j++) acc[j] = v[j];
            } else {
#pragma unroll
                for (int j = 0; j < CH_K; j++) acc[j] += v[j];
            }
        }
        if (NB > 0 && first_slab && warp == 0) {
            st_next_valid = vi + 1 < grp.n_voices;
            if (st_next_valid && lane < 4) st_next = insts[inst + 1].bq[0].state[lane];
        }
        if (handoff_in && warp == 0) {
            st_next_valid = false;
            if (vi + 1 < grp.n_voices) {
                if (lane == 0 && seen <= (unsigned)(vi + 1) && poll_ok(xa, vi + 1)) seen = xa & 0xfffffu;
                st_next_valid = __shfl_sync(0xffffffffu, seen > (unsigned)(vi + 1) ? 1 : 0, 0) != 0;
                if (st_next_valid && lane < 4) st_next = __ldcg(sc.handoff + ((size_t)(inst + 1) * 2 + (slab & 1)) * 4 + lane);
            }
        }
        __syncthreads();
        if (NB > 0 && t == PUB_T) {
            pe0 = sm.state[0][0]; pe1 = sm.state[0][1]; pe2 = sm.state[0][2]; pe3 = sm.state[0][3];
            pub_ptr = st_ptr;
            pub_vi = vi;
        }
    }
    if (NB > 0 && t == PUB_T) publish();
    (void)handoff_out;
    if (!active) return;
    const int64_t nabs = ci.f0 + n0;
    for (int oc = 0; oc < grp.out_dup; oc++) {
        float* out = chan(grp.out, oc, ci) + n0;
        if ((reinterpret_cast<uintptr_t>(out) & 15) == 0 && (grp.limit < 0 || nabs + CH_K <= grp.limit)) {
#pragma unroll
            for (int u = 0; u < CH_K / 4; u++) reinterpret_cast<float4*>(out)[u] = make_float4(acc[4 * u], acc[4 * u + 1], acc[4 * u + 2], acc[4 * u + 3]);
        } else {
#pragma unroll
            for (int j = 0; j < CH_K; j++)
                if (grp.limit < 0 || nabs + j < grp.limit) out[j] = acc[j];
        }
    }
}

__global__ void __launch_bounds__(256) k_osc_arate(const OscArInst* __restrict__ insts, int n_inst, ChunkInfo ci) {
    __shared__ double s_sum[256];
    __shared__ double s_carry;
    const OscArInst q = insts[blockIdx.x];
    const OscInst& o = q.base;
    float* out = chan(o.out, 0, ci);
    const float* ft = q.freq.p ? chan(q.freq, 0, ci) : nullptr;
    const float* dtk = q.detune.p ? chan(q.detune, 0, ci) : nullptr;
    const int t = threadIdx.x;
    const double sr = (double)q.sample_rate, nyq = sr / 2.;
    if (t == 0) s_carry = *q.phase;
    __syncthreads();
    for (int base = 0; base < ci.nf; base += 2048) {
        const int n0 = base + t * 8;
        double inc[8];
        bool act[8], oob[8];
        double local = 0.;
#pragma unroll
        for (int j = 0; j < 8; j++) {
            const int n = n0 + j;
            const int64_t na = ci.f0 + n;
            act[j] = n < ci.nf && na >= o.n_first && na < o.n_stop;
            double cf = 0.;
            if (n < ci.nf) {
                float f = ft ? ft[n] : q.f_val, d = dtk ? dtk[n] : q.d_val;
                cf = (double)f * exp2((double)d / 1200.);
            }
            oob[j] = fabs(cf) >= nyq;
            inc[j] = cf / sr;
            double add = act[j] ? inc[j] : 0.;
            if (act[j] && na == o.n_first) add += q.start_ratio * inc[j];
            local += add;
        }
        s_sum[t] = local;
        __syncthreads();
        for (int off = 1; off < 256; off <<= 1) {
            double v = t >= off ? s_sum[t - off] : 0.;
            __syncthreads();
            s_sum[t] += v;
            __syncthreads();
        }
        double ph = s_carry + (t > 0 ? s_sum[t - 1] : 0.);
        float v[8];
#pragma unroll
        for (int j = 0; j < 8; j++) {
            const int64_t na = ci.f0 + n0 + j;
            double p = ph;
            if (act[j] && na == o.n_first) p += q.start_ratio * inc[j];
            p -= floor(p);
            if (p >= 1.) p = 0.;
            v[j] = (act[j] && !oob[j]) ? osc_sample(o, p, inc[j]) : 0.f;
            if (act[j]) ph = p + inc[j];
        }
        if (n0 < ci.nf) {
            *reinterpret_cast<float4*>(out + n0) = make_float4(v[0], v[1], v[2], v[3]);
            *reinterpret_cast<float4*>(out + n0 + 4) = make_float4(v[4], v[5], v[6], v[7]);
        }
        __syncthreads();
        if (t == 255) {
            double c = s_carry + s_sum[255];
            s_carry = c - floor(c);
        }
        __syncthreads();
    }
    if (t == 0) *q.phase = s_carry;
}

struct BqC {
// ... 2729 lines not shown
        slabs = ((long)g_chain_waves * slots + ctas - 1) / ctas;
        if (slabs > tiles / min_tiles) slabs = tiles / min_tiles;
    }
    if (slabs > CHAIN_MAX_SLABS) slabs = CHAIN_MAX_SLABS;
    if (slabs < 1) slabs = 1;
    long tps = (tiles + slabs - 1) / slabs;
    if (tps < 1) tps = 1;
    slabs = (tiles + tps - 1) / tps;
    if (slabs < 1) slabs = 1;
    *n_slabs = (int)slabs;
    *tiles_per_slab = (int)tps;
}
template <int SRC, int NB>
static void launch_chain_v(bool shaper, const ChainInst* d, const ScanCoef* c, int n, int max_ch, ChunkInfo ci, cudaStream_t s, ChainAux aux) {
    ChainSched sc{};
    int pre_log2 = -1;
    chain_plan_slabs(n, max_ch, ci.nf, NB, &sc.n_slabs, &sc.tiles_per_slab, &pre_log2);
    if (NB > 0 && (sc.n_slabs > aux.slab_stride || !aux.ticket)) {
        sc.n_slabs = 1;
        sc.tiles_per_slab = (ci.nf + CH_THREADS * CH_K - 1) / (CH_THREADS * CH_K);
        pre_log2 = -1;
    }
    sc.pre_log2 = sc.n_slabs > 1 ? pre_log2 : -1;
    sc.max_ch = max_ch;
    sc.slab_stride = aux.slab_stride > 0 ? aux.slab_stride : 1;
    sc.epoch = aux.epoch;
    sc.ticket = (NB > 0 && sc.n_slabs > 1) ? aux.ticket : nullptr;
    sc.handoff = aux.handoff;
    sc.flags = aux.flags;
    const unsigned grid = (unsigned)n * (unsigned)max_ch * (unsigned)sc.n_slabs;
    constexpr bool STREAMED = SRC == CHAIN_SRC_BUFFER || SRC == CHAIN_SRC_ABSN;
    static bool carved = false;
    if (!carved && !getenv("WAE_CHAIN_NO_CARVEOUT")) {
        carved = true;
        cudaFuncSetAttribute(k_chain<SRC, NB, true, false>, cudaFuncAttributePreferredSharedMemoryCarveout, cudaSharedmemCarveoutMaxShared);
        cudaFuncSetAttribute(k_chain<SRC, NB, false, false>, cudaFuncAttributePreferredSharedMemoryCarveout, cudaSharedmemCarveoutMaxShared);
        if constexpr (STREAMED) {
            cudaFuncSetAttribute(k_chain<SRC, NB, true, true>, cudaFuncAttributePreferredSharedMemoryCarveout, cudaSharedmemCarveoutMaxShared);
            cudaFuncSetAttribute(k_chain<SRC, NB, false, true>, cudaFuncAttributePreferredSharedMemoryCarveout, cudaSharedmemCarveoutMaxShared);
        }
    }
    if constexpr (STREAMED) {
        if (g_chain_tma) {
            if (shaper) k_chain<SRC, NB, true, true><<<grid, CH_THREADS, 0, s>>>(d, c, n, ci, sc);
            else k_chain<SRC, NB, false, true><<<grid, CH_THREADS, 0, s>>>(d, c, n, ci, sc);
            return;
        }
    }
    if constexpr (NB == 1) {
        if (sc.pre_log2 >= 0) {
            static bool carved_pre = false;
            if (!carved_pre && !getenv("WAE_CHAIN_NO_CARVEOUT")) {
                carved_pre = true;
                cudaFuncSetAttribute(k_chain<SRC, NB, true, false, true>, cudaFuncAttributePreferredSharedMemoryCarveout, cudaSharedmemCarveoutMaxShared);
                cudaFuncSetAttribute(k_chain<SRC, NB, false, false, true>, cudaFuncAttributePreferredSharedMemoryCarveout, cudaSharedmemCarveoutMaxShared);
            }
            if (shaper) k_chain<SRC, NB, true, false, true><<<grid, CH_THREADS, 0, s>>>(d, c, n, ci, sc);
            else k_chain<SRC, NB, false, false, true><<<grid, CH_THREADS, 0, s>>>(d, c, n, ci, sc);
            return;
        }
    }
    {
        if (shaper) k_chain<SRC, NB, true, false><<<grid, CH_THREADS, 0, s>>>(d, c, n, ci, sc);
        else k_chain<SRC, NB, false, false><<<grid, CH_THREADS, 0, s>>>(d, c, n, ci, sc);
    }
}
template <int SRC>
static void launch_chain_s(int nb, bool shaper, const ChainInst* d, const ScanCoef* c, int n, int max_ch, ChunkInfo ci, cudaStream_t s, ChainAux aux) {
    if (nb == 0) launch_chain_v<SRC, 0>(shaper, d, c, n, max_ch, ci, s, aux);
    else if (nb == 1) launch_chain_v<SRC, 1>(shaper, d, c, n, max_ch, ci, s, aux);
    else launch_chain_v<SRC, 2>(shaper, d, c, n, max_ch, ci, s, aux);
}
void launch_chain(int variant, const ChainInst* d, const ScanCoef* c, int n, int max_ch, ChunkInfo ci, cudaStream_t s, ChainAux aux) {
    const int src = variant / 6, nb = (variant % 6) / 2;
    const bool shaper = (variant & 1) != 0;
    switch (src) {
        case CHAIN_SRC_BUFFER: launch_chain_s<CHAIN_SRC_BUFFER>(nb, shaper, d, c, n, max_ch, ci, s, aux); break;
        case CHAIN_SRC_ABSN: launch_chain_s<CHAIN_SRC_ABSN>(nb, shaper, d, c, n, max_ch, ci, s, aux); break;
        case CHAIN_SRC_OSC: launch_chain_s<CHAIN_SRC_OSC>(nb, shaper, d, c, n, max_ch, ci, s, aux); break;
        default: launch_chain_s<CHAIN_SRC_CONST>(nb, shaper, d, c, n, max_ch, ci, s, aux); break;
    }
}
int voice_sum_slots() { return g_num_sms * (WAE_VS_MINB * 128 / CH_THREADS); }
void launch_voice_sum(int nb, const ChainInst* d, const ScanCoef* c, const VoiceGroup* g, int n_groups, ChunkInfo ci, cudaStream_t s, ChainAux aux) {
    ChainSched sc{};
    const int n_tiles = (ci.nf + CH_THREADS * CH_K - 1) / (CH_THREADS * CH_K);
    sc.n_slabs = n_tiles;
    sc.tiles_per_slab = 1;
    sc.max_ch = 1;
    sc.slab_stride = aux.slab_stride;
    sc.epoch = aux.epoch;
    sc.pre_log2 = -1;
    sc.ticket = aux.ticket;
    sc.handoff = aux.handoff;
    sc.flags = aux.flags;
    const unsigned grid = (unsigned)n_tiles * (unsigned)n_groups;
    static bool carved = false;
    if (!carved) {
        carved = true;
        cudaFuncSetAttribute(k_voice_sum<0>, cudaFuncAttributePreferredSharedMemoryCarveout, cudaSharedmemCarveoutMaxShared);
        cudaFuncSetAttribute(k_voice_sum<1>, cudaFuncAttributePreferredSharedMemoryCarveout, cudaSharedmemCarveoutMaxShared);
    }
    if (nb == 0) k_voice_sum<0><<<grid, CH_THREADS, 0, s>>>(d, c, g, n_groups, ci, sc);
    else k_voice_sum<1><<<grid, CH_THREADS, 0, s>>>(d, c, g, n_groups, ci, sc);
}
void launch_iir(const IirInst* d, int n, int max_ch, ChunkInfo ci, cudaStream_t s) {
    int threads = n * max_ch;
    k_iir_serial<<<(threads + 63) / 64, 64, 0, s>>>(d, n, max_ch, ci);
}
void launch_gain(const GainInst* d, int n, ChunkInfo ci, cudaStream_t s) { k_gain<<<grid_tiles(ci.nf, 1024, n), 256, 0, s>>>(d, n, ci); }
void launch_shaper(const ShaperInst* d, int n, ChunkInfo ci, cudaStream_t s) { k_shaper<<<grid_tiles(ci.nf, 1024, n), 256, 0, s>>>(d, n, ci); }
void launch_stereo_panner(const SPanInst* d, const float2* g, int n, ChunkInfo ci, cudaStream_t s) {
    k_stereo_panner<<<grid_tiles(ci.nf, 256, n), 256, 0, s>>>(d, g, n, ci);
}
void launch_buffer_source_serial(const AbsnSerialInst* d, int n, ChunkInfo ci, cudaStream_t s) {
    k_buffer_source_serial<<<(n + ABSN_SERIAL_WARPS - 1) / ABSN_SERIAL_WARPS, 32 * ABSN_SERIAL_WARPS, 0, s>>>(d, n, ci);
}
void launch_shaper_os(const ShaperOsInst* d, int n, int max_ch, ChunkInfo ci, cudaStream_t s) {
    k_shaper_os_prev<<<(n + 63) / 64, 64, 0, s>>>(d, n, ci);
    k_shaper_os<<<dim3((unsigned)(ci.nf / 128), (unsigned)max_ch, (unsigned)n), 128, 0, s>>>(d, ci);
    k_shaper_os_hist<<<n, 256, 0, s>>>(d, ci);
}
void launch_panner_dyn(const PanDynInst* d, int n, ChunkInfo ci, cudaStream_t s) { k_panner_dyn<<<grid_tiles(ci.nf, 128, n), 128, 0, s>>>(d, n, ci); }
void launch_hrtf(const HrtfInst* d, int n, const HrtfSelInst* sel, int n_sel, int max_taps, ChunkInfo ci, cudaStream_t s) {
    if (n_sel > 0) k_hrtf_sel<<<dim3((ci.nf / 128 + 63) / 64 + 1, n_sel), 64, 0, s>>>(sel, ci);
    const int L4 = (max_taps + 3) & ~3;
    const int nx = 4 + (L4 - 1) + HRTF_TILE;
    const int copies = n_sel > 0 ? 8 : 1;
    const size_t smem = (size_t)(((nx + (nx >> 3) + 4) & ~3) + copies * 2 * L4) * sizeof(float);
    static size_t configured = 48 * 1024;
    if (smem > configured) {
        cudaFuncSetAttribute(k_hrtf_fir, cudaFuncAttributeMaxDynamicSharedMemorySize, (int)smem);
        configured = smem;
    }
    k_hrtf_map<<<(n + 63) / 64, 64, 0, s>>>(d, n, ci);
    k_hrtf_fir<<<dim3((ci.nf + HRTF_TILE - 1) / HRTF_TILE, n), 128, smem, s>>>(d, ci);
    k_hrtf_fill<<<grid_tiles(ci.nf, 256, n), 256, 0, s>>>(d, n, ci);
    k_hrtf_hist<<<n, 128, (size_t)max_taps * sizeof(float), s>>>(d, ci);
}
void launch_panner_eq(const PanInst* d, int n, ChunkInfo ci, cudaStream_t s) { k_panner_eq<<<grid_tiles(ci.nf, 256, n), 256, 0, s>>>(d, n, ci); }
void launch_route(const RouteInst* d, int n, ChunkInfo ci, cudaStream_t s) { k_route<<<grid_tiles(ci.nf, 1024, n), 256, 0, s>>>(d, n, ci); }
void launch_delay_read(const DelayInst* d, int n, ChunkInfo ci, cudaStream_t s) { k_delay_read<<<grid_tiles(ci.nf, 256, n), 256, 0, s>>>(d, n, ci); }
void launch_delay_mono(const DelayInst* d, int n, ChunkInfo ci, cudaStream_t s) { k_delay_mono<<<(n + 63) / 64, 64, 0, s>>>(d, n, ci); }
void launch_ring_write(const DelayInst* d, int n, ChunkInfo ci, cudaStream_t s) { k_ring_write<<<grid_tiles(ci.nf, 256, n), 256, 0, s>>>(d, n, ci); }
void launch_osc_arate(const OscArInst* d, int n, ChunkInfo ci, cudaStream_t s) { k_osc_arate<<<n, 256, 0, s>>>(d, n, ci); }
void launch_biquad_arate(const BiquadArInst* d, int n, int max_ch, ChunkInfo ci, cudaStream_t s) {
    k_biquad_coefs<<<grid_tiles(ci.nf, 256, n), 256, 0, s>>>(d, n, ci);
    const int warps = n * max_ch;
    k_biquad_arate<<<(warps + BQA_WARPS - 1) / BQA_WARPS, 32 * BQA_WARPS, 0, s>>>(d, n, max_ch, ci);
}
void launch_analyser_fft(const float* ring, uint32_t write_index, int fft_size, float smoothing, float* last_fft, float* out_db, cudaStream_t s) {
    static bool configured = false;
    if (!configured) {
        cudaFuncSetAttribute(k_analyser_fft, cudaFuncAttributeMaxDynamicSharedMemorySize, 16384 * (int)sizeof(float2));
        configured = true;
    }
    k_analyser_fft<<<1, 256, (size_t)(fft_size / 2) * sizeof(float2), s>>>(ring, write_index, fft_size, smoothing, last_fft, out_db);
}
void launch_readout_fft(const ReadoutInst* d, int n, int max_fft, ChunkInfo ci, cudaStream_t s) {
    static bool configured = false;
    if (!configured) {
        cudaFuncSetAttribute(k_readout_fft, cudaFuncAttributeMaxDynamicSharedMemorySize, 16384 * (int)sizeof(float2));
        configured = true;
    }
    k_readout_fft<<<n, 256, (size_t)(max_fft / 2) * sizeof(float2), s>>>(d, ci);
}
void launch_readout_time(const ReadoutInst* d, int n, int max_fft, ChunkInfo ci, cudaStream_t s) {
    k_readout_time<<<dim3(n, (max_fft + 255) / 256), 256, 0, s>>>(d, ci);
}
void launch_readout_smooth(const ReadoutSmoothInst* d, int n, int max_bins, ChunkInfo ci, cudaStream_t s) {
    k_readout_smooth<<<dim3(n, (max_bins + 255) / 256), 256, 0, s>>>(d, ci);
}
void launch_resample_linear(const float* in, int64_t len, float* out, int64_t target_len, cudaStream_t s) {
    k_resample_linear<<<(unsigned)((target_len + 255) / 256), 256, 0, s>>>(in, len, out, target_len);
}
void launch_param(const ParamInst* d, int n, ChunkInfo ci, cudaStream_t s, int mode) {
    if (mode >= 2) k_param_spec<<<n, 32 * PSPEC_WARPS, 0, s>>>(d, n, ci);
    else if (mode == 1) k_param_parallel<<<(n + PARAM_WARPS - 1) / PARAM_WARPS, 32 * PARAM_WARPS, 0, s>>>(d, n, ci);
    else k_param<<<(n + PARAM_WARPS - 1) / PARAM_WARPS, 32 * PARAM_WARPS, 0, s>>>(d, n, ci);
}
void launch_compressor(const CompInst* d, const CompReadoutInst* ro, int n, ChunkInfo ci, cudaStream_t s) {
    if (ro) k_compressor<true><<<(n + 31) / 32, 32, 0, s>>>(d, ro, n, ci);
    else k_compressor<false><<<(n + 31) / 32, 32, 0, s>>>(d, nullptr, n, ci);
}
void launch_analyser(const AnalyserInst* d, int n, ChunkInfo ci, cudaStream_t s) { k_analyser<<<grid_tiles(ci.nf, 256, n), 256, 0, s>>>(d, n, ci); }
static void conv_configure() {
    static bool configured = false;
// ... 88 lines not shown
```

web-audio-api-rs_b200/csrc/wae_kernels.h:

```cpp
#pragma once
#include "wae_device.h"

#include <cuda_runtime.h>

namespace wae {

constexpr int WAE_CHAIN_K = 16;
constexpr int WAE_CONV_BLOCK = 8192;
constexpr int WAE_CONV_SPEC = WAE_CONV_BLOCK;
constexpr int WAE_CONV_H_PAD_LO = 7;
constexpr int WAE_CONV_H_PAD = 7 + 16;
struct ScanCoef {
    double Pshfl[5][4];
    double Plane[32][4];
    double Pwarp[4];
    double GL[16];
};
constexpr int WAE_CHAIN_PRE_TILES = 16;

struct ScanM2 {
    double a, b, c, d;
};
WAE_HD ScanM2 scan_mul(const ScanM2& x, const ScanM2& y) {
    return ScanM2{x.a * y.a + x.b * y.c, x.a * y.b + x.b * y.d, x.c * y.a + x.d * y.c, x.c * y.b + x.d * y.d};
// ... 166 lines not shown
}
WAE_HD int64_t absn_fast_end(const SchedClock& clock, int64_t lq, int64_t n_start, double duration) {
    const double block_duration = clock.dt * 128.;
    const int64_t max_q = (lq - n_start) / 128 + 2;
    int64_t played = 0;
    double bt = 0.;
    while (played < max_q) {
        bt += block_duration;
        played++;
        if (bt >= duration) break;
    }
    return n_start + played * 128;
}

struct AbsnLoopPoints {
    double start, end;
    double actual_start, actual_end;
};
WAE_HD AbsnLoopPoints absn_loop_points(double loop_start, double loop_end, double buffer_duration) {
    AbsnLoopPoints p;
    p.start = loop_start < 0. ? 0. : (loop_start > buffer_duration ? buffer_duration : loop_start);
    p.end = (loop_end <= 0. || loop_end > buffer_duration) ? buffer_duration : loop_end;
    const bool custom = p.start >= 0. && p.end > 0. && p.start < p.end;
    p.actual_start = custom ? p.start : 0.;
    p.actual_end = custom ? p.end : buffer_duration;
    return p;
}

WAE_HD int32_t absn_loop_segments(double ls2, double le2, double step, int64_t n_first, int64_t n_end, double off, int64_t* seg_n,
                                  double* seg_bt, int32_t cap) {
    seg_n[0] = n_first;
    seg_bt[0] = off;
    int32_t k = 1;
    if (!(off < le2)) return k;
    const double len2 = le2 - ls2;
    int64_t m = 0;
    double v = off;
    bool entered = false;
    auto tz = [](double x) { return 3.0e-8 * (1.0 + fabs(x)); };
    while (n_first + m < n_end) {
        const double to_ls = v < ls2 - tz(ls2) ? (ls2 - tz(ls2) - v) / step : 0.;
        const double to_le = v < le2 - tz(le2) ? (le2 - tz(le2) - v) / step : 0.;
        const double skip = !entered ? (to_le < to_ls ? to_le : to_ls) : to_le;
        const int64_t adv = (int64_t)floor(skip);
        if (adv > 0) {
            v += (double)adv * step;
            m += adv;
            continue;
        }
        double w = v;
        if (almost_equal(w, le2)) w = le2;
        if (almost_equal(w, ls2)) w = ls2;
        if (!entered && w >= ls2) entered = true;
        if (entered) {
            while (w >= le2) w -= len2;
            while (w < ls2) w += len2;
        }
        if (w != v && n_first + m > seg_n[k - 1]) {
            if (k == cap) return -1;
            seg_n[k] = n_first + m;
            seg_bt[k] = w;
            k++;
        } else if (w != v) {
            seg_bt[k - 1] = w;
        }
        v = w + step;
        m += 1;
    }
    return k;
}

void upload_twiddles();
void conv_fft_selftest(float* data, int mode);
void launch_oscillator(const OscInst* d, int n, ChunkInfo ci, cudaStream_t s);
void launch_constant(const ConstInst* d, int n, ChunkInfo ci, cudaStream_t s);
void launch_buffer_source(const AbsnInst* d, int n, ChunkInfo ci, cudaStream_t s);
void launch_buffer_source_slow(const AbsnSlowInst* d, int n, ChunkInfo ci, cudaStream_t s);
void launch_buffer_source_bound(const AbsnBoundInst* d, int n, ChunkInfo ci, cudaStream_t s);
void launch_mix(const MixInst* d, const MixEdge* e, int n, ChunkInfo ci, cudaStream_t s, int max_edges);
void launch_mix_dyn(const MixDynInst* d, const MixEdge* e, int n, ChunkInfo ci, cudaStream_t s);
void launch_meta(const MetaInst* d, int n, ChunkInfo ci, cudaStream_t s);
void launch_biquad_serial(const BiquadInst* d, int n, int max_ch, ChunkInfo ci, cudaStream_t s);
void launch_chain(int variant, const ChainInst* d, const ScanCoef* c, int n, int max_ch, ChunkInfo ci, cudaStream_t s, ChainAux aux);
void launch_voice_sum(int nb, const ChainInst* d, const ScanCoef* c, const VoiceGroup* g, int n_groups, ChunkInfo ci, cudaStream_t s, ChainAux aux);
int voice_sum_slots();
void set_num_sms(int n);
void chain_plan_slabs(int n, int max_ch, int nf, int nb, int* n_slabs, int* tiles_per_slab, int* pre_log2 = nullptr);
void chain_set_prepass(int on);
void chain_set_tuning(int tma, int waves);
void launch_iir(const IirInst* d, int n, int max_ch, ChunkInfo ci, cudaStream_t s);
void launch_gain(const GainInst* d, int n, ChunkInfo ci, cudaStream_t s);
void launch_shaper(const ShaperInst* d, int n, ChunkInfo ci, cudaStream_t s);
void launch_stereo_panner(const SPanInst* d, const float2* gains, int n, ChunkInfo ci, cudaStream_t s);
void launch_hrtf(const HrtfInst* d, int n, const HrtfSelInst* sel, int n_sel, int max_taps, ChunkInfo ci, cudaStream_t s);
void launch_buffer_source_serial(const AbsnSerialInst* d, int n, ChunkInfo ci, cudaStream_t s);
void launch_shaper_os(const ShaperOsInst* d, int n, int max_ch, ChunkInfo ci, cudaStream_t s);
void launch_panner_dyn(const PanDynInst* d, int n, ChunkInfo ci, cudaStream_t s);
void launch_panner_eq(const PanInst* d, int n, ChunkInfo ci, cudaStream_t s);
void launch_route(const RouteInst* d, int n, ChunkInfo ci, cudaStream_t s);
void launch_delay_read(const DelayInst* d, int n, ChunkInfo ci, cudaStream_t s);
void launch_delay_mono(const DelayInst* d, int n, ChunkInfo ci, cudaStream_t s);
void launch_ring_write(const DelayInst* d, int n, ChunkInfo ci, cudaStream_t s);
void launch_osc_arate(const OscArInst* d, int n, ChunkInfo ci, cudaStream_t s);
void launch_biquad_arate(const BiquadArInst* d, int n, int max_ch, ChunkInfo ci, cudaStream_t s);
void launch_analyser_fft(const float* ring, uint32_t write_index, int fft_size, float smoothing, float* last_fft, float* out_db, cudaStream_t s);
void launch_resample_linear(const float* in, int64_t len, float* out, int64_t target_len, cudaStream_t s);
void launch_param(const ParamInst* d, int n, ChunkInfo ci, cudaStream_t s, int mode);
void launch_compressor(const CompInst* d, const CompReadoutInst* ro, int n, ChunkInfo ci, cudaStream_t s);
void launch_analyser(const AnalyserInst* d, int n, ChunkInfo ci, cudaStream_t s);
void launch_readout_fft(const ReadoutInst* d, int n, int max_fft, ChunkInfo ci, cudaStream_t s);
void launch_readout_time(const ReadoutInst* d, int n, int max_fft, ChunkInfo ci, cudaStream_t s);
void launch_readout_smooth(const ReadoutSmoothInst* d, int n, int max_bins, ChunkInfo ci, cudaStream_t s);
void launch_conv_fft_in(const ConvInput* d, int n, ChunkInfo ci, cudaStream_t s);
void launch_conv_mac_ifft(const ConvPath* p, const ConvInput* in, int n, ChunkInfo ci, cudaStream_t s);
void launch_conv_compact(const ConvCmpInst* d, int n, ChunkInfo ci, cudaStream_t s);
void launch_bind_sources(const BindItem* d, int n, int64_t max_vec, int max_ch, cudaStream_t s);
void launch_bind_params(const ParamBindItem* d, int n, const ParamSlotInfo* info, float* values, const ParamPatch* patches, int n_patches,
                        cudaStream_t s);
void launch_derive_spatial(const SpatialPatch* patches, int n, const float* values, const RespBindItem* resp, int n_resp, int max_taps,
                           int max_S, cudaStream_t s);
void launch_bind_responses(RespBindItem* d, int n, bool any_normalize, int64_t max_len, int max_S, int max_ch, cudaStream_t s);
void launch_bind_curves(const CurveBindItem* d, int n, cudaStream_t s);
void launch_bind_waves(const WaveBindItem* d, int n, int max_len, bool any_normalize, cudaStream_t s);
void launch_bind_iir(const IirBindItem* d, int n, cudaStream_t s);
void launch_bind_value_curves(const ValueCurveBindItem* d, int n, int64_t max_len, cudaStream_t s);
void launch_bind_schedules(const SchedBindItem* d, int n, cudaStream_t s);
void launch_bind_loops(const LoopBindItem* d, int n, cudaStream_t s);
void launch_absn_loop_schedule(const LoopWalk* d, int n, int* overflow, cudaStream_t s);
void launch_bind_output(const OutPatch* d, int n, float* base, cudaStream_t s);
void launch_bind_source_refs(const SrcRefBindItem* d, int n, const SrcRefPatch* entries, cudaStream_t s);
void launch_conv_ir_fft(const float* ir, int64_t ir_len, int64_t ir_stride, float2* h, int S, int channels, cudaStream_t s);

}
```

Before: 1.374 billion.

## Split voice-sum into a state pre-pass and an independent per-tile sum kernel

Replaces the ticketed, flag-polling serial hand-off of biquad state between tiles inside the voice-sum kernel with two launches. First a state-only k_chain pass runs per voice and records the filter state at each tile boundary, skipping output writes. Then the voice-sum kernel reads those per-tile states and processes all tiles fully in parallel. This removes inter-block spin-waiting and ticket ordering, at the cost of an extra launch, a second pass over the oscillator source and recurrence, and extra device memory for the tile states, which also feeds into chunk sizing.

```diff
diff --git a/web-audio-api-rs_b200/csrc/wae_device.h b/web-audio-api-rs_b200/csrc/wae_device.h
--- a/web-audio-api-rs_b200/csrc/wae_device.h
+++ b/web-audio-api-rs_b200/csrc/wae_device.h
@@ -436,6 +436,9 @@
     unsigned* ticket;
     double* handoff;
     unsigned* flags;
+    double* tile_states;
+    int32_t states_stride;
+    int32_t pad;
 };
 struct ChainAux {
     unsigned* ticket = nullptr;
@@ -443,6 +446,8 @@
     unsigned* flags = nullptr;
     int32_t slab_stride = 0;
     uint32_t epoch = 0;
+    double* tile_states = nullptr;
+    int32_t states_stride = 0;
 };
 
 struct VoiceGroup {
diff --git a/web-audio-api-rs_b200/csrc/wae_engine.cu b/web-audio-api-rs_b200/csrc/wae_engine.cu
--- a/web-audio-api-rs_b200/csrc/wae_engine.cu
+++ b/web-audio-api-rs_b200/csrc/wae_engine.cu
@@ -1003,6 +1003,7 @@
         return vs_mode;
     }
     uint64_t arena_floats_per_frame = 0;
+    uint64_t state_voices = 0;
     float* d_src = nullptr;
     std::vector<wae_batch::Group::SrcCopy>* src_copies = nullptr;
     size_t src_cursor = 0;
@@ -1100,6 +1101,7 @@
         builds.clear();
         arena_used.clear();
         arena_floats_per_frame = 0;
+        state_voices = 0;
     }
     template <typename T>
     T* upload(const std::vector<T>& v) {
@@ -2236,6 +2238,7 @@
         vs.chain.push_back(pc.inst);
     }
     vs.vgroups.push_back(vg);
+    if (nb > 0) state_voices += edges.size();
     if (nc.n.kind == K_DEST) add_out(vs, offsetof(VoiceGroup, out), T_C);
     nc.p.in_buf[port] = vg.out;
     return true;
@@ -3928,8 +3931,9 @@
     uint64_t fpf = 0;
     bool has_feedback = false;
     std::vector<std::vector<int>> plan_stage_lists;
+    uint64_t svf = 0;
     struct SizeOut {
-        uint64_t fpf = 0;
+        uint64_t fpf = 0, svf = 0;
         bool has_feedback = false;
         std::map<std::pair<uint32_t, uint32_t>, int> delay_ch_seen;
         std::vector<std::vector<int>> stage_lists;
@@ -3943,10 +3947,11 @@
     for (int iter = 0; iter < 8; iter++) {
         bool hints_changed = false;
         fpf = 0;
+        svf = 0;
         plan_stage_lists.clear();
         std::vector<SizeOut> so(n_groups);
         struct RangeOut {
-            uint64_t fpf = 0;
+            uint64_t fpf = 0, svf = 0;
             size_t src_floats = 0;
             bool has_feedback = false;
             std::map<std::pair<uint32_t, uint32_t>, int> delay_ch_seen;
@@ -3971,6 +3976,7 @@
             }
             if (plan) ro.builds = std::move(sizing.builds);
             ro.fpf = sizing.arena_floats_per_frame;
+            ro.svf = sizing.state_voices;
             ro.src_floats = sizing.src_cursor - cursor0;
             ro.has_feedback = sizing.has_feedback;
             ro.delay_ch_seen = std::move(sizing.delay_ch_seen);
@@ -3996,6 +4002,7 @@
                 for (size_t gb : r.graph_base) out.graph_base.push_back(gb + rebase);
                 if (plan) merge_builds(out.builds, r.builds);
                 out.fpf += r.fpf;
+                out.svf += r.svf;
                 out.src_floats += r.src_floats;
                 out.has_feedback = out.has_feedback || r.has_feedback;
                 for (auto& kv : r.delay_ch_seen) out.delay_ch_seen[kv.first] = kv.second;
@@ -4023,6 +4030,7 @@
                 b->groups[k].graph_src_base = std::move(out.graph_base);
                 b->groups[k].src_floats = out.src_floats;
                 so[k].fpf = out.fpf;
+                so[k].svf = out.svf;
                 so[k].has_feedback = out.has_feedback;
                 so[k].delay_ch_seen = std::move(out.delay_ch_seen);
                 return;
@@ -4045,6 +4053,7 @@
                     }
                 }
                 so[k].fpf = std::max(so[k].fpf, sizing.arena_floats_per_frame);
+                so[k].svf = std::max(so[k].svf, sizing.state_voices);
                 if (plan) {
                     std::vector<int> kinds;
                     for (auto& kv : sizing.builds) kinds.push_back(kv.second.kind);
@@ -4067,7 +4076,7 @@
                 static const bool threaded = [] { const char* e = getenv("WAE_PLAN_PARALLEL"); return e && atoi(e) >= 2; }();
                 std::unique_ptr<WorkerPool> tmp_pool(threaded ? new WorkerPool(3, 0) : nullptr);
                 const bool ok = size_group_split(k, tmp_pool.get(), (int)std::min<uint32_t>(n_in_group, 3u), out);
-                bool same = ok && out.fpf == so[k].fpf && out.src_floats == b->groups[k].src_floats && out.has_feedback == so[k].has_feedback &&
+                bool same = ok && out.fpf == so[k].fpf && out.svf == so[k].svf && out.src_floats == b->groups[k].src_floats && out.has_feedback == so[k].has_feedback &&
                             out.delay_ch_seen == so[k].delay_ch_seen && out.copies.size() == b->groups[k].src_copies.size() &&
                             out.graph_base == b->groups[k].graph_src_base;
                 if (same) {
@@ -4098,6 +4107,7 @@
                 return fail(code, msg);
             }
             fpf = std::max(fpf, so[k].fpf);
+            svf = std::max(svf, so[k].svf);
             has_feedback = has_feedback || so[k].has_feedback;
             for (auto& l : so[k].stage_lists) plan_stage_lists.push_back(std::move(l));
             if (plan && plan_digest_wanted()) {
@@ -4127,10 +4137,10 @@
     b->asset_bytes = 0;
     int64_t chunk = eng->chunk_frames;
     if (chunk == 0) {
-        if (fpf == 0) {
+        if (fpf == 0 && svf == 0) {
             chunk = b->lq;
         } else {
-            chunk = (int64_t)(1024.0 * 1024 * 1024 / (4.0 * (double)fpf));
+            chunk = (int64_t)(1024.0 * 1024 * 1024 / (4.0 * (double)fpf + 32.0 / 2048 * (double)svf));
             chunk = std::max<int64_t>(8192, std::min<int64_t>(chunk, 1 << 20));
             chunk = chunk / 2048 * 2048;
         }
@@ -4317,13 +4327,20 @@
                 }
                 case S_VSUM: {
                     st.n = (int)s.vgroups.size(); st.d_a = up(b, s.chain); st.d_b = up(b, s.scan_coef); st.d_c = up(b, s.vgroups);
-                    const int64_t nf_max = std::min<int64_t>(b->chunk, pl.seg_end - pl.seg_start);
-                    const int tiles = (int)((nf_max + 2047) / 2048);
-                    st.chain.slab_stride = tiles;
-                    st.chain.ticket = b->dalloc<unsigned>(1, true);
-                    st.chain.flags = b->dalloc<unsigned>((size_t)st.n * tiles, true);
-                    st.chain.handoff = b->dalloc<double>(s.chain.size() * 2 * 4);
-                    if (!st.chain.ticket || !st.chain.flags || !st.chain.handoff) return oom("voice-sum hand-off");
+                    st.n_b = (int)s.chain.size();
+                    if (s.variant > 0) {
+                        const int64_t nf_max = std::min<int64_t>(b->chunk, pl.seg_end - pl.seg_start);
+                        const int tiles = (int)((nf_max + 2047) / 2048);
+                        const int slabs = voice_sum_state_slabs(st.n_b, (int)nf_max);
+                        const size_t slots = (size_t)st.n_b * slabs;
+                        st.chain.slab_stride = slabs;
+                        st.chain.ticket = b->dalloc<unsigned>(1, true);
+                        st.chain.flags = b->dalloc<unsigned>(slots, true);
+                        st.chain.handoff = b->dalloc<double>(slots * CHAIN_MAX_BIQUADS * 4);
+                        st.chain.states_stride = tiles;
+                        st.chain.tile_states = b->dalloc<double>((size_t)st.n_b * tiles * 4);
+                        if (!st.chain.ticket || !st.chain.flags || !st.chain.handoff || !st.chain.tile_states) return oom("voice-sum states");
+                    }
                     break;
                 }
                 case S_PARAM: st.n = (int)s.param.size(); st.d_a = up(b, s.param); break;
@@ -4605,7 +4622,8 @@
     }
     uint64_t launches = 0;
     for (auto& st : b->stages) {
-        const uint64_t k = (st.kind == S_CONV_FFT || st.kind == S_CONV_MAC || st.kind == S_CONV_MAC_ACC || st.kind == S_SHAPER_OS) ? 2
+        const uint64_t k = (st.kind == S_CONV_FFT || st.kind == S_CONV_MAC || st.kind == S_CONV_MAC_ACC || st.kind == S_SHAPER_OS ||
+                            (st.kind == S_VSUM && st.variant > 0)) ? 2
                            : st.kind == S_HRTF ? (st.n_b > 0 ? 3 : 2) : st.kind == S_CONV_CMP ? 6 : 1;
         const std::vector<int64_t>& sb = b->groups[st.group].seg_bounds;
         const int64_t seg_len = sb[st.seg + 1] - sb[st.seg];
@@ -4811,7 +4829,7 @@
             break;
         case S_VSUM:
             st.chain.epoch++;
-            launch_voice_sum(st.variant, (ChainInst*)st.d_a, (ScanCoef*)st.d_b, (VoiceGroup*)st.d_c, st.n, ci, s, st.chain);
+            launch_voice_sum(st.variant, (ChainInst*)st.d_a, (ScanCoef*)st.d_b, (VoiceGroup*)st.d_c, st.n, st.n_b, ci, s, st.chain);
             break;
         case S_IIR: launch_iir((IirInst*)st.d_a, st.n, st.max_ch, ci, s); break;
         case S_GAIN: launch_gain((GainInst*)st.d_a, st.n, ci, s); break;
diff --git a/web-audio-api-rs_b200/csrc/wae_kernels.cu b/web-audio-api-rs_b200/csrc/wae_kernels.cu
--- a/web-audio-api-rs_b200/csrc/wae_kernels.cu
+++ b/web-audio-api-rs_b200/csrc/wae_kernels.cu
@@ -1105,7 +1105,7 @@
 template <typename RL>
 DEVI void chain_biquad(ChainSmem& sm, int bq, const double b0, const double b1, const double b2, const double a1, const double a2,
                        const double* Plane, float v[CH_K], bool active, int n_active, int t, int lane, int warp, bool want_clean, bool& clean,
-                       RL reload) {
+                       RL reload, const bool outputs = true) {
     const double* Psh = sm.P[bq];
     const double* Pw = sm.P[bq] + 20;
     const float xl1 = active ? v[CH_K - 1] : 0.f, xl2 = active ? v[CH_K - 2] : 0.f;
@@ -1174,16 +1174,18 @@
         mat2_fma(Plane, wa, wb, e1, e2);
     }
     if (want_clean) clean = !(x_normal || isnormal_d(e1) || isnormal_d(e2));
+    const bool last = active && t == n_active - 1;
     r1 = e1;
     r2 = e2;
-#pragma unroll
-    for (int j = 0; j < CH_K; j++) {
-        const double y = fma(na1, r1, fma(na2, r2, w[j]));
-        r2 = r1;
-        r1 = y;
-        v[j] = (float)y;
-    }
-    const bool last = active && t == n_active - 1;
+    if (outputs || last) {
+#pragma unroll
+        for (int j = 0; j < CH_K; j++) {
+            const double y = fma(na1, r1, fma(na2, r2, w[j]));
+            r2 = r1;
+            r1 = y;
+            if (outputs) v[j] = (float)y;
+        }
+    }
     const bool poisoned = last && (!(fabs(r1) <= 1.7976931348623157e308) || !(fabs(r2) <= 1.7976931348623157e308));
 #ifdef WAE_CHAIN_NOCHECK
     __syncthreads();
@@ -1308,7 +1310,7 @@
     const int base = src == CHAIN_SRC_OSC ? WAE_CH_MINB_OSC : WAE_CH_MINB;
     return ((nb == 2 ? base - 1 : base) * 128) / CH_THREADS;
 }
-template <int SRC, int NB, bool SHAPER, bool TMA, bool PRE = false>
+template <int SRC, int NB, bool SHAPER, bool TMA, bool PRE = false, bool STATES = false>
 __global__ void __launch_bounds__(CH_THREADS, chain_min_blocks(SRC, NB)) k_chain(const ChainInst* __restrict__ insts, const ScanCoef* __restrict__ coefs,
                                                                         int n_inst, ChunkInfo ci, ChainSched sc) {
     __shared__ ChainSmem sm;
@@ -1487,6 +1489,7 @@
     }
     int buf = 0;
     for (int base = slab_begin; base < slab_end; base += tile) {
+        if (STATES && t < 4) __stcg(sc.tile_states + ((size_t)inst * sc.states_stride + base / tile) * 4 + t, sm.state[0][t]);
         const int n0 = base + t * CH_K;
         const bool active = n0 < ci.nf;
         const int n_active = min(CH_THREADS, (ci.nf - base) / CH_K);
@@ -1549,7 +1552,8 @@
                 };
                 chain_biquad(sm, 0, cb[0][0], cb[0][1], cb[0][2], cb[0][3], cb[0][4], sm.plane[0][lane > 0 ? lane - 1 : 0], v, active, n_active, t, lane, warp, want_clean, clean0, reload);
             } else {
-                chain_biquad(sm, 0, cb[0][0], cb[0][1], cb[0][2], cb[0][3], cb[0][4], sm.plane[0][lane > 0 ? lane - 1 : 0], v, active, n_active, t, lane, warp, want_clean, clean0, NoReload{});
+                chain_biquad(sm, 0, cb[0][0], cb[0][1], cb[0][2], cb[0][3], cb[0][4], sm.plane[0][lane > 0 ? lane - 1 : 0], v, active, n_active, t, lane, warp, want_clean, clean0, NoReload{},
+                             !STATES);
             }
             if (g1 != 1.f) {
 #pragma unroll
@@ -1710,7 +1714,7 @@
             __syncthreads();
         }
     }
-    run_slab(true);
+    run_slab(!STATES);
     if (USE_TMA && t == 0) bulk_wait_read<0>();
     if (NB > 0) {
         if (last_slab) {
@@ -1732,18 +1736,11 @@
 template <int NB>
 __global__ void __launch_bounds__(CH_THREADS, WAE_VS_MINB * 128 / CH_THREADS) k_voice_sum(const ChainInst* __restrict__ insts, const ScanCoef* __restrict__ coefs,
                                                                                           const VoiceGroup* __restrict__ groups, int n_groups, ChunkInfo ci,
-                                                                                          ChainSched sc) {
+                                                                                          const double* __restrict__ states, int states_stride) {
     __shared__ ChainSmem sm;
-    __shared__ int s_item;
     __shared__ float2 s_table2[2048];
     const int t = threadIdx.x, lane = t & 31, warp = t >> 5;
-    if (t == 0) {
-        const unsigned tk = atomicAdd(sc.ticket, 1u);
-        if (tk == gridDim.x - 1) atomicExch(sc.ticket, 0u);
-        s_item = (int)tk;
-    }
-    __syncthreads();
-    const int item = s_item;
+    const int item = (int)blockIdx.x;
     const int slab = item / n_groups, gi = item - slab * n_groups;
     const VoiceGroup grp = groups[gi];
     constexpr int tile = CH_THREADS * CH_K;
@@ -1752,11 +1749,7 @@
     const int n0 = base + t * CH_K;
     const bool active = n0 < ci.nf;
     const int n_active = min(CH_THREADS, (ci.nf - base) / CH_K);
-    const bool first_slab = slab == 0, last_slab = base + tile >= ci.nf;
-    const unsigned tag = (sc.epoch & 0xfffu) << 20;
-    const unsigned* prog_prev = sc.flags + (size_t)gi * sc.slab_stride + (slab > 0 ? slab - 1 : 0);
-    unsigned* prog_mine = sc.flags + (size_t)gi * sc.slab_stride + slab;
-    unsigned seen = 0;
+    const bool past_end = ci.f0 + base >= insts[grp.first].end;
     const float* cur_table = nullptr;
     float acc[CH_K];
 #pragma unroll
@@ -1765,7 +1758,7 @@
     constexpr int PL_W = (128 + CH_THREADS - 1) / CH_THREADS;
     static_assert(CH_THREADS >= 24, "scan constants: one of Pshfl / Pwarp per thread");
     int rec_n[REC_W];
-    double pl_n[PL_W], pw_n = 0.;
+    double pl_n[PL_W], pw_n = 0., st_n = 0.;
     auto prefetch = [&](int vi) {
         const int inst = grp.first + vi;
         const int* src = reinterpret_cast<const int*>(insts + inst);
@@ -1777,31 +1770,11 @@
             for (int i = 0; i < PL_W; i++) pl_n[i] = (t + i * CH_THREADS) < 128 ? (&scf.Plane[0][0])[t + i * CH_THREADS] : 0.;
             if (t < 20) pw_n = (&scf.Pshfl[0][0])[t];
             else if (t < 24) pw_n = scf.Pwarp[t - 20];
+            if (t < 4 && !past_end) st_n = __ldg(states + ((size_t)inst * states_stride + slab) * 4 + t);
         }
     };
     prefetch(0);
-    const bool handoff_in = NB > 0 && !first_slab, handoff_out = NB > 0 && !last_slab;
-    auto poll_ok = [&](unsigned x, int v) { return (x & 0xfff00000u) == tag && (x & 0xfffffu) > (unsigned)v; };
-    double st_next = 0.;
-    bool st_next_valid = false;
-    constexpr int PUB_T = CH_WARPS > 1 ? 32 : 0;
-    double pe0 = 0., pe1 = 0., pe2 = 0., pe3 = 0.;
-    double* pub_ptr = nullptr;
-    int pub_vi = -1;
-    auto publish = [&]() {
-        if (pub_vi < 0) return;
-        if (last_slab) {
-            pub_ptr[0] = pe0; pub_ptr[1] = pe1; pub_ptr[2] = pe2; pub_ptr[3] = pe3;
-        } else {
-            double* dst = sc.handoff + ((size_t)(grp.first + pub_vi) * 2 + ((slab + 1) & 1)) * 4;
-            asm volatile("st.global.cg.v2.f64 [%0], {%1, %2};" ::"l"(dst), "d"(pe0), "d"(pe1) : "memory");
-            asm volatile("st.global.cg.v2.f64 [%0], {%1, %2};" ::"l"(dst + 2), "d"(pe2), "d"(pe3) : "memory");
-            asm volatile("st.release.gpu.global.u32 [%0], %1;" ::"l"(prog_mine), "r"(tag | (unsigned)(pub_vi + 1)) : "memory");
-        }
-        pub_vi = -1;
-    };
     for (int vi = 0; vi < grp.n_voices; vi++) {
-        const int inst = grp.first + vi;
 #pragma unroll
         for (int i = 0; i < REC_W; i++)
             if ((t + i * CH_THREADS) < (int)(sizeof(ChainInst) / 4)) reinterpret_cast<int*>(&sm.q)[t + i * CH_THREADS] = rec_n[i];
@@ -1810,36 +1783,11 @@
             for (int i = 0; i < PL_W; i++)
                 if ((t + i * CH_THREADS) < 128) (&sm.plane[0][0][0])[t + i * CH_THREADS] = pl_n[i];
             if (t < 24) sm.P[0][t] = pw_n;
+            if (t < 4) sm.state[0][t] = st_n;
         }
         __syncthreads();
         if (vi + 1 < grp.n_voices) prefetch(vi + 1);
         const ChainInst& q = sm.q;
-        double st_cur = 0.;
-        unsigned xa = 0;
-        if (NB > 0 && t == PUB_T) publish();
-        if (NB > 0 && warp == 0) {
-            if (st_next_valid) {
-                st_cur = st_next;
-            } else if (first_slab) {
-                if (lane < 4) st_cur = q.bq[0].state[lane];
-            } else {
-                if (lane == 0 && seen <= (unsigned)vi) {
-                    for (;;) {
-                        unsigned x;
-                        asm volatile("ld.relaxed.gpu.global.u32 %0, [%1];" : "=r"(x) : "l"(prog_prev) : "memory");
-                        if (poll_ok(x, vi)) {
-                            seen = x & 0xfffffu;
-                            break;
-                        }
-                        __nanosleep(20);
-                    }
-                }
-                __syncwarp();
-                if (lane < 4) st_cur = __ldcg(sc.handoff + ((size_t)inst * 2 + (slab & 1)) * 4 + lane);
-            }
-            if (handoff_in && lane == 0 && vi + 1 < grp.n_voices && seen <= (unsigned)(vi + 1))
-                asm volatile("ld.relaxed.gpu.global.u32 %0, [%1];" : "=r"(xa) : "l"(prog_prev));
-        }
         const float2* tab2 = nullptr;
         if ((q.osc.type == 0 || q.osc.type == 4) && q.osc.table_len == 2048) {
             if (q.osc.table != cur_table) {
@@ -1850,13 +1798,6 @@
             }
             tab2 = s_table2;
         }
-        double cb[5] = {0., 0., 0., 0., 0.};
-        double* st_ptr = nullptr;
-        if (NB > 0) {
-            const ChainBiquad& bq = q.bq[0];
-            cb[0] = bq.b0; cb[1] = bq.b1; cb[2] = bq.b2; cb[3] = bq.a1; cb[4] = bq.a2;
-            st_ptr = bq.state;
-        }
         const float g0 = q.g[0], g1 = q.g[1];
         float v[CH_K];
         if (active) chain_load_source<CHAIN_SRC_OSC>(q, 0, ci, n0, v, tab2);
@@ -1865,9 +1806,9 @@
             for (int j = 0; j < CH_K; j++) v[j] *= g0;
         }
         if (NB > 0) {
-            if (warp == 0 && lane < 4) sm.state[0][lane] = st_cur;
+            const ChainBiquad& bq = q.bq[0];
             bool clean = true;
-            chain_biquad(sm, 0, cb[0], cb[1], cb[2], cb[3], cb[4], sm.plane[0][lane > 0 ? lane - 1 : 0], v, active, n_active, t, lane, warp, false, clean, NoReload{});
+            chain_biquad(sm, 0, bq.b0, bq.b1, bq.b2, bq.a1, bq.a2, sm.plane[0][lane > 0 ? lane - 1 : 0], v, active, n_active, t, lane, warp, false, clean, NoReload{});
             if (g1 != 1.f) {
 #pragma unroll
                 for (int j = 0; j < CH_K; j++) v[j] *= g1;
@@ -1882,27 +1823,8 @@
                 for (int j = 0; j < CH_K; j++) acc[j] += v[j];
             }
         }
-        if (NB > 0 && first_slab && warp == 0) {
-            st_next_valid = vi + 1 < grp.n_voices;
-            if (st_next_valid && lane < 4) st_next = insts[inst + 1].bq[0].state[lane];
-        }
-        if (handoff_in && warp == 0) {
-            st_next_valid = false;
-            if (vi + 1 < grp.n_voices) {
-                if (lane == 0 && seen <= (unsigned)(vi + 1) && poll_ok(xa, vi + 1)) seen = xa & 0xfffffu;
-                st_next_valid = __shfl_sync(0xffffffffu, seen > (unsigned)(vi + 1) ? 1 : 0, 0) != 0;
-                if (st_next_valid && lane < 4) st_next = __ldcg(sc.handoff + ((size_t)(inst + 1) * 2 + (slab & 1)) * 4 + lane);
-            }
-        }
         __syncthreads();
-        if (NB > 0 && t == PUB_T) {
-            pe0 = sm.state[0][0]; pe1 = sm.state[0][1]; pe2 = sm.state[0][2]; pe3 = sm.state[0][3];
-            pub_ptr = st_ptr;
-            pub_vi = vi;
-        }
-    }
-    if (NB > 0 && t == PUB_T) publish();
-    (void)handoff_out;
+    }
     if (!active) return;
     const int64_t nabs = ci.f0 + n0;
     for (int oc = 0; oc < grp.out_dup; oc++) {
@@ -4798,27 +4720,42 @@
     }
 }
 int voice_sum_slots() { return g_num_sms * (WAE_VS_MINB * 128 / CH_THREADS); }
-void launch_voice_sum(int nb, const ChainInst* d, const ScanCoef* c, const VoiceGroup* g, int n_groups, ChunkInfo ci, cudaStream_t s, ChainAux aux) {
-    ChainSched sc{};
+int voice_sum_state_slabs(int n, int nf) {
+    int slabs = 1, tps = 1;
+    chain_plan_slabs(n, 1, nf, 1, &slabs, &tps);
+    return slabs;
+}
+void launch_voice_sum(int nb, const ChainInst* d, const ScanCoef* c, const VoiceGroup* g, int n_groups, int n_voices, ChunkInfo ci, cudaStream_t s,
+                      ChainAux aux) {
     const int n_tiles = (ci.nf + CH_THREADS * CH_K - 1) / (CH_THREADS * CH_K);
-    sc.n_slabs = n_tiles;
-    sc.tiles_per_slab = 1;
-    sc.max_ch = 1;
-    sc.slab_stride = aux.slab_stride;
-    sc.epoch = aux.epoch;
-    sc.pre_log2 = -1;
-    sc.ticket = aux.ticket;
-    sc.handoff = aux.handoff;
-    sc.flags = aux.flags;
-    const unsigned grid = (unsigned)n_tiles * (unsigned)n_groups;
     static bool carved = false;
     if (!carved) {
         carved = true;
+        cudaFuncSetAttribute(k_chain<CHAIN_SRC_OSC, 1, false, false, false, true>, cudaFuncAttributePreferredSharedMemoryCarveout, cudaSharedmemCarveoutMaxShared);
         cudaFuncSetAttribute(k_voice_sum<0>, cudaFuncAttributePreferredSharedMemoryCarveout, cudaSharedmemCarveoutMaxShared);
         cudaFuncSetAttribute(k_voice_sum<1>, cudaFuncAttributePreferredSharedMemoryCarveout, cudaSharedmemCarveoutMaxShared);
     }
-    if (nb == 0) k_voice_sum<0><<<grid, CH_THREADS, 0, s>>>(d, c, g, n_groups, ci, sc);
-    else k_voice_sum<1><<<grid, CH_THREADS, 0, s>>>(d, c, g, n_groups, ci, sc);
+    if (nb > 0) {
+        ChainSched sc{};
+        chain_plan_slabs(n_voices, 1, ci.nf, 1, &sc.n_slabs, &sc.tiles_per_slab);
+        if (sc.n_slabs > aux.slab_stride || !aux.ticket) {
+            sc.n_slabs = 1;
+            sc.tiles_per_slab = n_tiles;
+        }
+        sc.pre_log2 = -1;
+        sc.max_ch = 1;
+        sc.slab_stride = aux.slab_stride > 0 ? aux.slab_stride : 1;
+        sc.epoch = aux.epoch;
+        sc.ticket = sc.n_slabs > 1 ? aux.ticket : nullptr;
+        sc.handoff = aux.handoff;
+        sc.flags = aux.flags;
+        sc.tile_states = aux.tile_states;
+        sc.states_stride = aux.states_stride;
+        k_chain<CHAIN_SRC_OSC, 1, false, false, false, true><<<(unsigned)n_voices * (unsigned)sc.n_slabs, CH_THREADS, 0, s>>>(d, c, n_voices, ci, sc);
+    }
+    const unsigned grid = (unsigned)n_tiles * (unsigned)n_groups;
+    if (nb == 0) k_voice_sum<0><<<grid, CH_THREADS, 0, s>>>(d, c, g, n_groups, ci, nullptr, 0);
+    else k_voice_sum<1><<<grid, CH_THREADS, 0, s>>>(d, c, g, n_groups, ci, aux.tile_states, aux.states_stride);
 }
 void launch_iir(const IirInst* d, int n, int max_ch, ChunkInfo ci, cudaStream_t s) {
     int threads = n * max_ch;
diff --git a/web-audio-api-rs_b200/csrc/wae_kernels.h b/web-audio-api-rs_b200/csrc/wae_kernels.h
--- a/web-audio-api-rs_b200/csrc/wae_kernels.h
+++ b/web-audio-api-rs_b200/csrc/wae_kernels.h
@@ -272,8 +272,10 @@
 void launch_meta(const MetaInst* d, int n, ChunkInfo ci, cudaStream_t s);
 void launch_biquad_serial(const BiquadInst* d, int n, int max_ch, ChunkInfo ci, cudaStream_t s);
 void launch_chain(int variant, const ChainInst* d, const ScanCoef* c, int n, int max_ch, ChunkInfo ci, cudaStream_t s, ChainAux aux);
-void launch_voice_sum(int nb, const ChainInst* d, const ScanCoef* c, const VoiceGroup* g, int n_groups, ChunkInfo ci, cudaStream_t s, ChainAux aux);
+void launch_voice_sum(int nb, const ChainInst* d, const ScanCoef* c, const VoiceGroup* g, int n_groups, int n_voices, ChunkInfo ci, cudaStream_t s,
+                      ChainAux aux);
 int voice_sum_slots();
+int voice_sum_state_slabs(int n_voices, int nf);
 void set_num_sms(int n);
 void chain_plan_slabs(int n, int max_ch, int nf, int nb, int* n_slabs, int* tiles_per_slab, int* pre_log2 = nullptr);
 void chain_set_prepass(int on);
```

New measurement: 1.374 billion (median of 6 runs). No clear change (-0.0%).
